# EnricoMiccoli/nodal

Hardware: NVIDIA B200
Metric: unknowns_per_second (higher is better)
Workload: dtype f64

## Files before the change

__graft_entry__.py:

```python
import os
import subprocess
import sys

ROOT = os.path.dirname(os.path.abspath(__file__))
if ROOT not in sys.path:
    sys.path.insert(0, ROOT)


def build():
    subprocess.check_call(["make", "-C", os.path.join(ROOT, "nodal_b200", "csrc"), "-j8"])
    sys.path.insert(0, os.path.join(ROOT, "tests"))
    import helpers
    helpers.stamp_host_lib()
    helpers.amg_host_lib()
    import sources_host
    sources_host.sources_host_lib()
    import amg_cycle_host
    amg_cycle_host.amg_cycle_host_lib()
    ref_nodal = os.path.join(os.environ.get("NODAL_REFERENCE", "/root/reference"), "nodal")
    if os.path.isdir(ref_nodal) and not os.path.isfile(os.path.join(ROOT, "baseline", "_ref", "nodal", "nodal.py")):
        subprocess.call([sys.executable, os.path.join(ROOT, "baseline", "install_ref.py")])
    import nodal_b200
    from nodal_b200 import _lib
    _lib.load()


def smoke():
    import numpy as np
    import nodal_b200 as n
    import nodal_b200.equiv
    from nodal_b200 import dist as ndist
    from nodal_b200 import generators as gen
    from nodal_b200.device import Device
    from oracle import mna_oracle as orc

    N = 24
    r_cpu = orc.equivalent_resistance(orc.grid2d_rows(N), "1", "g", sparse=True, backend="dict")
    r_gpu = n.equiv.equivalent_resistance(gen.grid2d(N), "1", "g", sparse=True)
    r_jac = n.equiv.equivalent_resistance(gen.grid2d(N), "1", "g", sparse=True, precond="jacobi")
    r_amg = n.equiv.equivalent_resistance(gen.grid2d(N), "1", "g", sparse=True, precond="amg", amg={"coarse": 64})
    for r in (r_gpu, r_jac, r_amg):
        assert abs(r - r_cpu) <= 1e-9 * abs(r_cpu), (r, r_cpu)
    dev = Device.get(0)
    import copy
    net = copy.deepcopy(gen.grid2d(64))
    net.process_component(["a1", "A", "1", "1", "g"])
    table = net.table()
    csr, rhs = dev.assemble_csr(table)
    x, info = ndist.single_solver(dev).solve_amg(csr.n, np.array([0, csr.n], dtype=np.int32), csr.indptr, csr.indices,
                                                  csr.data, rhs, rtol=1e-10, gather_below=300)
    r_dist = float(x[net.nodenum["1"]])
    r64 = orc.equivalent_resistance(orc.grid2d_rows(64), "1", "g", sparse=True, backend="dict")
    assert info["status"] == 0 and info["distributed_levels"] >= 1 and abs(r_dist - r64) <= 1e-9 * abs(r64), (info, r_dist, r64)
    pg = gen.power_grid(16, 5, vdd=1.0, load=1e-3, seed=0)
    sol = n.Circuit(pg, sparse=True, eliminate_sources=True).solve()
    red = sol.stats["reduction"]
    assert red["eliminated"] and red["relres_full"] <= 1e-9 and np.all(sol.potentials() <= 1.0), sol.stats
    print(f"smoke ok: R({N}x{N} grid) default={float(r_gpu)!r} jacobi={float(r_jac)!r} amg={float(r_amg)!r} "
          f"oracle={float(r_cpu)!r}; R(64x64) partitioned-AMG form={r_dist!r} oracle={float(r64)!r}; "
          f"power grid 16x16 relres_full={red['relres_full']:.1e}")


if __name__ == "__main__":
    build()
    if len(sys.argv) > 1 and sys.argv[1] == "smoke":
        smoke()
```

include/nodal_b200.h:

```cpp
#ifndef NODAL_B200_H
#define NODAL_B200_H

#include <stdint.h>

#ifdef __cplusplus
extern "C" {
#endif

#define NODAL_ABI_VERSION 1

enum {
    NODAL_OK = 0,
    NODAL_SINGULAR = 1,
    NODAL_NOT_CONVERGED = 2,
    NODAL_BREAKDOWN = 3,
    NODAL_CUDA_ERROR = 4,
    NODAL_BAD_ARG = -1
};

enum { NODAL_T_R = 0, NODAL_T_A = 1, NODAL_T_E = 2, NODAL_T_VCVS = 3, NODAL_T_VCCS = 4,
       NODAL_T_CCVS = 5, NODAL_T_CCCS = 6 };
#define NODAL_GROUND (-1)
#define NODAL_UNUSED (-2)

typedef struct nodal_ctx nodal_ctx;

int nodal_abi_version(void);
const char* nodal_last_error(void);
uint64_t nodal_launch_count(void);
int nodal_ctx_create(int device, nodal_ctx** out);
int nodal_ctx_destroy(nodal_ctx* ctx);
int64_t nodal_ctx_workspace_bytes(nodal_ctx* ctx);

int nodal_stamp_coo(nodal_ctx* ctx, int64_t ncomp,
                    const uint8_t* type, const double* value,
                    const int32_t* a, const int32_t* b, const int32_t* c, const int32_t* d,
                    const int32_t* drv, const int32_t* branch,
                    int32_t kcl, int32_t n, int32_t stride, int32_t colbits,
                    uint64_t* keys, double* vals, void* stream);

int nodal_csr_build(nodal_ctx* ctx, int32_t n, int64_t nslots, int32_t colbits,
                    uint64_t* keys, double* vals, double* rhs,
                    int64_t* nnz_h, void* stream);
int nodal_csr_fetch(nodal_ctx* ctx, int32_t n, int64_t nnz,
                    int32_t* indptr, int32_t* indices, double* data, void* stream);
int nodal_csr_build_ordered(nodal_ctx* ctx, int32_t n, int64_t nslots, int32_t colbits,
                            uint64_t* keys, double* vals, int32_t order, double* rhs, int64_t* nnz_h,
                            void* stream);

int nodal_csr_to_dense(nodal_ctx* ctx, int32_t n, const int32_t* indptr, const int32_t* indices,
                       const double* data, double* G, void* stream);
int nodal_coo_to_dense_atomic(nodal_ctx* ctx, int32_t n, int64_t nslots, int32_t colbits,
                              const uint64_t* keys, const double* vals, double* G, double* rhs,
                              void* stream);

int nodal_spmv(nodal_ctx* ctx, int32_t n, int64_t nnz, const int32_t* indptr,
               const int32_t* indices, const double* data, const double* x, double* y,
               void* stream);

typedef struct nodal_sell nodal_sell;
int nodal_sell_create(nodal_ctx* ctx, int32_t n, int64_t nnz, const int32_t* indptr,
                      const int32_t* indices, const double* data, nodal_sell** out, void* stream);
int nodal_sell_destroy(nodal_sell* m);
int64_t nodal_sell_padded_nnz(const nodal_sell* m);
int nodal_sell_spmv(nodal_ctx* ctx, const nodal_sell* m, const double* x, double* y, void* stream);

int nodal_pcg(nodal_ctx* ctx, int32_t n, int64_t nnz, const int32_t* indptr,
              const int32_t* indices, const double* data, const double* rhs, double* x,
              double rtol, int32_t maxit, int32_t flags,
              int32_t* iters_h, double* relres_h, double* stats_h, void* stream);
#define NODAL_PCG_FORCE_CSR 1
#define NODAL_PCG_NO_GRAPH 2
#define NODAL_PCG_PROFILE 4
#define NODAL_PCG_NO_SCALE 8

int nodal_gmres(nodal_ctx* ctx, int32_t n, int64_t nnz, const int32_t* indptr,
                const int32_t* indices, const double* data, const double* rhs, double* x,
                double rtol, int32_t restart, int32_t maxit,
                int32_t* iters_h, double* relres_h, void* stream);

typedef struct nodal_amg nodal_amg;
int nodal_amg_create(nodal_ctx* ctx, int32_t n, int64_t nnz, const int32_t* indptr,
                     const int32_t* indices, const double* data, const double* params,
                     nodal_amg** out, void* stream);
int nodal_amg_destroy(nodal_amg* amg);
int nodal_amg_info(const nodal_amg* amg, int32_t cap, int32_t* nlevels, int64_t* rows, int64_t* nnz,
                   double* setup_ms, int32_t* direct);
int nodal_amg_fetch_level(nodal_ctx* ctx, const nodal_amg* amg, int32_t level, int32_t* agg,
                          int32_t* indptr, int32_t* indices, double* data, void* stream);
int nodal_amg_apply(nodal_ctx* ctx, const nodal_amg* amg, const double* r, double* z, void* stream);
int nodal_amg_pcg(nodal_ctx* ctx, nodal_amg* amg, const double* rhs, double* x, double rtol,
                  int32_t maxit, int32_t* iters_h, double* relres_h, double* stats_h, void* stream);

int nodal_connected_components(nodal_ctx* ctx, int64_t ncomp, const int32_t* a, const int32_t* b,
                               int32_t kcl, int32_t* labels, int32_t* ncomponents_h,
                               int32_t* reached_h, void* stream);

int nodal_source_forest(nodal_ctx* ctx, int64_t ncomp, const uint8_t* type, const double* value,
                        const int32_t* a, const int32_t* b, const int32_t* branch, int32_t kcl, int32_t be,
                        int32_t* erow, int32_t* adj_ptr, int32_t* adj_row, int32_t* rep_row, double* offset,
                        int32_t* parent_edge, int32_t* depth, int32_t* roots, int64_t* info_h, void* stream);
int nodal_source_reduce_scan(nodal_ctx* ctx, int64_t ncomp, const uint8_t* type, const int32_t* a,
                             const int32_t* b, int32_t kcl, const int32_t* rep_row, const double* offset,
                             uint32_t* pos, int64_t* count_h, void* stream);
int nodal_source_reduce_table(nodal_ctx* ctx, int64_t ncomp, const uint8_t* type, const double* value,
                              const int32_t* a, const int32_t* b, int32_t kcl, const int32_t* rep_row,
                              const double* offset, const uint32_t* pos, uint8_t* out_type, double* out_value,
                              int32_t* out_a, int32_t* out_b, void* stream);
int nodal_source_expand(nodal_ctx* ctx, int32_t kcl, int32_t n, int32_t nsrc, const int32_t* erow,
                        const int32_t* a, const int32_t* b, const int32_t* branch, const int32_t* adj_ptr,
                        const int32_t* adj_row, const int32_t* rep_row, const double* offset,
                        const int32_t* depth, int32_t max_depth, const double* y, const double* rhs,
                        int64_t nnz, const int32_t* indptr, const int32_t* indices, const double* data,
                        double* x, double* relres_h, void* stream);
int nodal_source_potentials(nodal_ctx* ctx, int32_t kcl, int32_t n, const int32_t* rep_row, const double* offset,
                            const double* y, double* x, void* stream);
int nodal_source_tree_rows(nodal_ctx* ctx, int32_t kcl, int32_t n, int64_t nnz_full, int32_t rb, int32_t re,
                           const int32_t* depth, const double* rhs, int64_t nnz, const int32_t* indptr,
                           const int32_t* indices, const double* data, const double* x, int32_t* out_row,
                           double* out_rhs, double* out_gx, int64_t* count_h, void* stream);
int nodal_source_currents(nodal_ctx* ctx, int32_t kcl, int32_t nsrc, const int32_t* erow, const int32_t* a,
                          const int32_t* b, const int32_t* branch, const int32_t* adj_ptr, const int32_t* adj_row,
                          const int32_t* depth, int32_t max_depth, int64_t ntree, const int32_t* tree_row,
                          const double* tree_rhs, const double* tree_gx, double* x, void* stream);
int nodal_source_residual(nodal_ctx* ctx, int32_t n, int64_t nnz_full, int32_t rows, const double* rhs, int64_t nnz,
                          const int32_t* indptr, const int32_t* indices, const double* data, const double* x,
                          double* sums_h, void* stream);

int nodal_lu_solve(nodal_ctx* ctx, int32_t n, double* G, const double* rhs, double* x,
                   int32_t* info_h, void* stream);

int nodal_dgemm_sub_profile(nodal_ctx* ctx, double* C, const double* A, const double* B, int32_t M, int32_t N,
                            int32_t K, int32_t ld, int32_t reps, double* ms_out, void* stream);

int nodal_lu_batched(nodal_ctx* ctx, int64_t batch, int32_t ncomp,
                     const uint8_t* type, const int32_t* a, const int32_t* b,
                     const int32_t* c, const int32_t* d, const int32_t* drv, const int32_t* branch,
                     int32_t kcl, int32_t n, const double* values, double* x, int32_t* info,
                     void* stream);

int nodal_lu_batched_soa(nodal_ctx* ctx, int64_t batch, int32_t ncomp,
                         const uint8_t* type, const int32_t* a, const int32_t* b,
                         const int32_t* c, const int32_t* d, const int32_t* drv, const int32_t* branch,
                         int32_t kcl, int32_t n, const double* values_t, double* x_t, int32_t* info,
                         void* stream);

typedef struct nodal_dist nodal_dist;
int nodal_dist_unique_id(uint8_t id_h[128]);
// ... 54 lines not shown
```

nodal_b200/_lib.py:

```python
from __future__ import annotations

import ctypes as C
import os

_HERE = os.path.dirname(os.path.abspath(__file__))
LIB_PATH = os.path.join(_HERE, "libnodal_b200.so")

OK, SINGULAR, NOT_CONVERGED, BREAKDOWN, CUDA_ERROR, BAD_ARG = 0, 1, 2, 3, 4, -1
PCG_FORCE_CSR, PCG_NO_GRAPH, PCG_PROFILE, PCG_NO_SCALE = 1, 2, 4, 8

_vp, _i32, _i64, _f64 = C.c_void_p, C.c_int32, C.c_int64, C.c_double

SIGNATURES = {
    "nodal_abi_version": (C.c_int, []),
    "nodal_last_error": (C.c_char_p, []),
    "nodal_launch_count": (C.c_uint64, []),
    "nodal_ctx_create": (C.c_int, [C.c_int, C.POINTER(_vp)]),
    "nodal_ctx_destroy": (C.c_int, [_vp]),
    "nodal_ctx_workspace_bytes": (_i64, [_vp]),
    "nodal_stamp_coo": (C.c_int, [_vp, _i64, _vp, _vp, _vp, _vp, _vp, _vp, _vp, _vp,
                                  _i32, _i32, _i32, _i32, _vp, _vp, _vp]),
    "nodal_csr_build": (C.c_int, [_vp, _i32, _i64, _i32, _vp, _vp, _vp, C.POINTER(_i64), _vp]),
    "nodal_csr_build_ordered": (C.c_int, [_vp, _i32, _i64, _i32, _vp, _vp, _i32, _vp, C.POINTER(_i64), _vp]),
    "nodal_csr_fetch": (C.c_int, [_vp, _i32, _i64, _vp, _vp, _vp, _vp]),
    "nodal_csr_to_dense": (C.c_int, [_vp, _i32, _vp, _vp, _vp, _vp, _vp]),
    "nodal_coo_to_dense_atomic": (C.c_int, [_vp, _i32, _i64, _i32, _vp, _vp, _vp, _vp, _vp]),
    "nodal_spmv": (C.c_int, [_vp, _i32, _i64, _vp, _vp, _vp, _vp, _vp, _vp]),
    "nodal_sell_create": (C.c_int, [_vp, _i32, _i64, _vp, _vp, _vp, C.POINTER(_vp), _vp]),
    "nodal_sell_destroy": (C.c_int, [_vp]),
    "nodal_sell_padded_nnz": (_i64, [_vp]),
    "nodal_sell_spmv": (C.c_int, [_vp, _vp, _vp, _vp, _vp]),
    "nodal_pcg": (C.c_int, [_vp, _i32, _i64, _vp, _vp, _vp, _vp, _vp, _f64, _i32, _i32,
                            C.POINTER(_i32), C.POINTER(_f64), C.POINTER(_f64), _vp]),
    "nodal_gmres": (C.c_int, [_vp, _i32, _i64, _vp, _vp, _vp, _vp, _vp, _f64, _i32, _i32,
                              C.POINTER(_i32), C.POINTER(_f64), _vp]),
    "nodal_amg_create": (C.c_int, [_vp, _i32, _i64, _vp, _vp, _vp, C.POINTER(_f64), C.POINTER(_vp), _vp]),
    "nodal_amg_destroy": (C.c_int, [_vp]),
    "nodal_amg_info": (C.c_int, [_vp, _i32, C.POINTER(_i32), C.POINTER(_i64), C.POINTER(_i64),
                                 C.POINTER(_f64), C.POINTER(_i32)]),
    "nodal_amg_fetch_level": (C.c_int, [_vp, _vp, _i32, _vp, _vp, _vp, _vp, _vp]),
    "nodal_amg_apply": (C.c_int, [_vp, _vp, _vp, _vp, _vp]),
    "nodal_amg_pcg": (C.c_int, [_vp, _vp, _vp, _vp, _f64, _i32, C.POINTER(_i32), C.POINTER(_f64),
                                C.POINTER(_f64), _vp]),
    "nodal_connected_components": (C.c_int, [_vp, _i64, _vp, _vp, _i32, _vp, C.POINTER(_i32),
                                             C.POINTER(_i32), _vp]),
    "nodal_source_forest": (C.c_int, [_vp, _i64, _vp, _vp, _vp, _vp, _vp, _i32, _i32] + [_vp] * 8
                            + [C.POINTER(_i64), _vp]),
    "nodal_source_reduce_scan": (C.c_int, [_vp, _i64, _vp, _vp, _vp, _i32, _vp, _vp, _vp, C.POINTER(_i64), _vp]),
    "nodal_source_reduce_table": (C.c_int, [_vp, _i64, _vp, _vp, _vp, _vp, _i32, _vp, _vp, _vp, _vp, _vp, _vp, _vp,
                                            _vp]),
    "nodal_source_expand": (C.c_int, [_vp, _i32, _i32, _i32] + [_vp] * 9 + [_i32, _vp, _vp, _i64, _vp, _vp, _vp, _vp,
                                                                             C.POINTER(_f64), _vp]),
    "nodal_lu_solve": (C.c_int, [_vp, _i32, _vp, _vp, _vp, C.POINTER(_i32), _vp]),
    "nodal_dgemm_sub_profile": (C.c_int, [_vp, _vp, _vp, _vp, _i32, _i32, _i32, _i32, _i32, C.POINTER(_f64), _vp]),
    "nodal_lu_batched": (C.c_int, [_vp, _i64, _i32, _vp, _vp, _vp, _vp, _vp, _vp, _vp,
                                   _i32, _i32, _vp, _vp, _vp, _vp]),
    "nodal_lu_batched_soa": (C.c_int, [_vp, _i64, _i32, _vp, _vp, _vp, _vp, _vp, _vp, _vp,
                                       _i32, _i32, _vp, _vp, _vp, _vp]),
    "nodal_dist_unique_id": (C.c_int, [_vp]),
    "nodal_dist_create": (C.c_int, [_vp, _vp, _i32, _i32, C.POINTER(_vp)]),
    "nodal_dist_create_single": (C.c_int, [_vp, C.POINTER(_vp)]),
    "nodal_dist_destroy": (C.c_int, [_vp]),
    "nodal_dist_pcg": (C.c_int, [_vp, _vp, _i32, _vp, _i64, _vp, _vp, _vp, _vp, _vp, _f64, _i32,
                                 C.POINTER(_i32), C.POINTER(_f64), C.POINTER(_f64), _vp]),
    "nodal_amg_pcg_multi": (C.c_int, [_vp, _vp, _i32, _vp, _vp, _f64, _i32, C.POINTER(_i32), C.POINTER(_f64),
                                      C.POINTER(_i32), _vp]),
    "nodal_amg_profile_sweeps": (C.c_int, [_vp, _vp, _i32, C.POINTER(_f64), _vp]),
    "nodal_amg_profile_cycle": (C.c_int, [_vp, _vp, _i32, C.POINTER(_f64), _vp]),
    "nodal_table_select_scan": (C.c_int, [_vp, _i64, _vp, _vp, _i32, _i32, _vp, C.POINTER(_i64), _vp]),
    "nodal_table_select_gather": (C.c_int, [_vp, _i64, _vp, _i32, _i32] + [_vp] * 16 + [_vp]),
    "nodal_table_select_mna_scan": (C.c_int, [_vp, _i64, _vp, _vp, _vp, _vp, _i32, _i32, _i32, _vp, C.POINTER(_i64),
                                              _vp]),
    "nodal_table_select_mna_gather": (C.c_int, [_vp, _i64, _vp, _i32, _i32, _i32] + [_vp] * 16 + [_vp]),
    "nodal_table_select_type_scan": (C.c_int, [_vp, _i64, _vp, _vp, _vp, _i32, _vp, C.POINTER(_i64), _vp]),
    "nodal_table_select_type_gather": (C.c_int, [_vp, _i64, _vp, _i32] + [_vp] * 16 + [_vp]),
    "nodal_source_potentials": (C.c_int, [_vp, _i32, _i32, _vp, _vp, _vp, _vp, _vp]),
    "nodal_source_tree_rows": (C.c_int, [_vp, _i32, _i32, _i64, _i32, _i32, _vp, _vp, _i64, _vp, _vp, _vp, _vp, _vp,
                                         _vp, _vp, C.POINTER(_i64), _vp]),
    "nodal_source_currents": (C.c_int, [_vp, _i32, _i32] + [_vp] * 7 + [_i32, _i64, _vp, _vp, _vp, _vp, _vp]),
    "nodal_source_residual": (C.c_int, [_vp, _i32, _i64, _i32, _vp, _i64, _vp, _vp, _vp, _vp, C.POINTER(_f64), _vp]),
    "nodal_dist_amg_pcg": (C.c_int, [_vp, _vp, _i32, _vp, _i64, _vp, _vp, _vp, _vp, _vp, C.POINTER(_f64), _f64,
                                     _i32, C.POINTER(_i32), C.POINTER(_f64), C.POINTER(_f64), _vp]),
}

_lib = None


class NodalLibraryError(RuntimeError):
    """The CUDA extension is missing or a CUDA call failed."""


def load():
    global _lib
    if _lib is not None:
        return _lib
    if not os.path.exists(LIB_PATH):
        raise NodalLibraryError(
            f"{LIB_PATH} not found: build it with `python -c 'import __graft_entry__ as g; g.build()'`"
            " (or `make -C nodal_b200/csrc`). nodal_b200 has no CPU fallback.")
    lib = C.CDLL(LIB_PATH)
    for name, (res, args) in SIGNATURES.items():
        fn = getattr(lib, name)
        fn.restype = res
        fn.argtypes = args
    if lib.nodal_abi_version() != 1:
        raise NodalLibraryError("libnodal_b200.so ABI version mismatch")
    _lib = lib
    return lib


def last_error():
    return load().nodal_last_error().decode("utf-8", "replace")


# ... 5 lines not shown
```

nodal_b200/csrc/amg.cu:

```cuda
#include <algorithm>
#include <cmath>

#include "amg_host.cuh"

void amg_free_csr(nodal_ctx* ctx, AmgCsr& a) {
    if (a.owned) {
        ctx_pool_free(ctx, const_cast<int32_t*>(a.indptr));
        ctx_pool_free(ctx, const_cast<int32_t*>(a.indices));
        ctx_pool_free(ctx, const_cast<double*>(a.data));
    }
    a = AmgCsr();
}

int amg_aggregate(nodal_ctx* ctx, int rounds, const AmgCsr& A, int32_t nown, int32_t base,
                  int32_t** agg_out, int32_t* nc_out, cudaStream_t st) {
    const int32_t n = A.n;
    AmgScratch<int32_t> match(ctx, n), best(ctx, n);
    AmgScratch<u32> leader(ctx, n);
    if (!match.ptr || !best.ptr || !leader.ptr) return NODAL_CUDA_ERROR;
    const int grid = amg_rows_grid(ctx, n);
    CUDA_TRY(cudaMemsetAsync(match, 0xFF, sizeof(int32_t) * (size_t)n, st));
    for (int r = 0; r < rounds; ++r) {
        amg_propose_kernel<<<grid, AT, 0, st>>>(n, A.indptr, A.indices, A.data, match, best, nown, base);
        KERNEL_CHECK();
// ... 187 lines not shown
        nodal_set_error("amg: the coarsest operator is not positive definite (pivot %d of %d); "
                        "the matrix is not SPD", *bad_h, n);
        return NODAL_BREAKDOWN;
    }
    return NODAL_OK;
}

int build_hierarchy(nodal_amg* h, int32_t n, int64_t nnz, const int32_t* indptr, const int32_t* indices,
                    const double* data, cudaStream_t st) {
    nodal_ctx* ctx = h->ctx;
    Csr cur;
    cur.n = n; cur.nnz = nnz; cur.indptr = indptr; cur.indices = indices; cur.data = data;
    while (cur.n > h->coarse && (int)h->lv.size() < h->maxlevels) {
        Csr A = cur;
        A.owned = false;
        int32_t* comp = nullptr;
        int rc = NODAL_OK;
        for (int pass = 0; pass < h->passes && rc == NODAL_OK; ++pass) {
            int32_t* agg = nullptr;
            int32_t nc = 0;
            Csr Ac;
            rc = aggregate(h, A, &agg, &nc, st);
            if (rc == NODAL_OK) rc = galerkin(h, A, agg, nc, &Ac, st);
            if (rc == NODAL_OK && comp) {
                amg_compose_kernel<<<rows_grid(ctx, cur.n), AT, 0, st>>>(cur.n, comp, agg);
                ++g_nodal_launches;
                if (cudaGetLastError() != cudaSuccess) {
                    nodal_set_error("amg: amg_compose_kernel launch failed");
                    rc = NODAL_CUDA_ERROR;
                }
            }
            if (!comp) comp = agg;
            else ctx_pool_free(ctx, agg);
            free_csr(ctx, A);
            A = Ac;
        }
        double total_nnz = (double)cur.nnz + (double)A.nnz;
        for (const AmgLevel& P : h->lv) total_nnz += (double)P.nnz;
        const bool too_dense = (double)A.nnz > h->max_fill * (double)cur.nnz ||
                               total_nnz > h->max_complexity * (double)(h->lv.empty() ? cur.nnz : h->lv[0].nnz);
        if (rc != NODAL_OK || (double)A.n > 0.9 * (double)cur.n || too_dense) {
            free_csr(ctx, A);
            ctx_pool_free(ctx, comp);
            if (rc != NODAL_OK) {
                free_csr(ctx, cur);
                return rc;
            }
            break;
        }
        AmgLevel L;
        L.n = cur.n; L.nnz = cur.nnz; L.indptr = cur.indptr; L.indices = cur.indices; L.data = cur.data;
        L.owned = cur.owned;
        L.agg = comp;
        L.nc = A.n;
        h->lv.push_back(L);
        cur = A;
        rc = transpose_pattern(h, h->lv.back(), st);
        if (rc != NODAL_OK) {
            free_csr(ctx, cur);
            return rc;
        }
    }
    AmgLevel L;
    L.n = cur.n; L.nnz = cur.nnz; L.indptr = cur.indptr; L.indices = cur.indices; L.data = cur.data;
    L.owned = cur.owned;
    h->lv.push_back(L);
    for (size_t l = 0; l < h->lv.size(); ++l) {
        AmgLevel& V = h->lv[l];
        NODAL_TRY(sell_from_csr(ctx, V.n, V.nnz, V.indptr, V.indices, V.data, &V.sell, st, nullptr));
        V.x = pool<double>(ctx, V.n);
        V.r = pool<double>(ctx, V.n);
        if (l > 0) V.b = pool<double>(ctx, V.n);
        if (!V.x || !V.r || (l > 0 && !V.b)) return NODAL_CUDA_ERROR;
    }
    if (h->lv.back().n <= h->direct_max) NODAL_TRY(invert_coarsest(h, h->lv.back(), st));
    return NODAL_OK;
}

template <int MODE>
int sell_sweep(const nodal_amg* h, const AmgLevel& V, const double* b, const double* x, double* y,
               double* part, cudaStream_t st) {
    const nodal_sell* m = V.sell;
    amg_sell_kernel<MODE><<<sell_grid(h->ctx, m->nslices), AT, 0, st>>>(
        m->n, m->nslices, m->slice_w, m->cols, m->vals, m->dinv, b, x, h->omega, y, part);
    KERNEL_CHECK();
    return NODAL_OK;
}

template <int MODE>
int cycle_sweep(const nodal_amg* h, const AmgLevel& V, const double* b, const double* xc, double* y,
                cudaStream_t st) {
    const nodal_sell* m = V.sell;
    amg_cycle_sweep_kernel<MODE><<<sell_grid(h->ctx, m->nslices), AT, 0, st>>>(
        m->n, m->nslices, m->slice_w, m->cols, m->vals, m->dinv, b, h->omega, V.agg, xc, h->scale, y);
    KERNEL_CHECK();
    return NODAL_OK;
}

int cycle(const nodal_amg* h, const double* b0, double* z0, cudaStream_t st) {
    const nodal_ctx* ctx = h->ctx;
    const int last = (int)h->lv.size() - 1;
    for (int l = 0; l < last; ++l) {
        const AmgLevel& V = h->lv[l];
        const double* b = l == 0 ? b0 : V.b;
        NODAL_TRY(cycle_sweep<1>(h, V, b, nullptr, V.r, st));
        amg_restrict_kernel<<<rows_grid(ctx, V.nc), AT, 0, st>>>(V.nc, V.pt_ptr, V.pt_idx, V.r,
                                                              h->lv[l + 1].b);
        KERNEL_CHECK();
    }
    {
        const AmgLevel& V = h->lv[last];
        const double* b = last == 0 ? b0 : V.b;
        double* x = last == 0 ? z0 : V.x;
        if (h->inv) amg_gemv_kernel<<<rows_grid(ctx, (int64_t)V.n * 32), AT, 0, st>>>(V.n, h->inv, b, x);
        else amg_jacobi0_kernel<<<rows_grid(ctx, V.n), AT, 0, st>>>(V.n, V.sell->dinv, b, h->omega, x);
        KERNEL_CHECK();
    }
    for (int l = last - 1; l >= 0; --l) {
        const AmgLevel& V = h->lv[l];
        const double* b = l == 0 ? b0 : V.b;
        NODAL_TRY(cycle_sweep<2>(h, V, b, h->lv[l + 1].x, l == 0 ? z0 : V.x, st));
    }
    return NODAL_OK;
}

}

extern "C" int nodal_amg_destroy(nodal_amg* h) {
    if (!h) return NODAL_OK;
    cudaSetDevice(h->device);
    nodal_ctx* ctx = h->ctx;
    for (AmgLevel& V : h->lv) {
        sell_free(V.sell);
        if (V.owned) {
            ctx_pool_free(ctx, const_cast<int32_t*>(V.indptr));
            ctx_pool_free(ctx, const_cast<int32_t*>(V.indices));
            ctx_pool_free(ctx, const_cast<double*>(V.data));
        }
        ctx_pool_free(ctx, V.agg);
        ctx_pool_free(ctx, V.pt_ptr);
        ctx_pool_free(ctx, V.pt_idx);
        ctx_pool_free(ctx, V.b);
        ctx_pool_free(ctx, V.x);
        ctx_pool_free(ctx, V.r);
    }
    ctx_pool_free(ctx, h->inv);
    ctx_pool_free(ctx, h->p);
    ctx_pool_free(ctx, h->q);
    ctx_pool_free(ctx, h->r);
    ctx_pool_free(ctx, h->z);
    ctx_pool_free(ctx, h->part);
    delete h;
    return NODAL_OK;
}

extern "C" int nodal_amg_create(nodal_ctx* ctx, int32_t n, int64_t nnz, const int32_t* indptr,
                                const int32_t* indices, const double* data, const double* params,
                                nodal_amg** out, void* stream) {
    NvtxRange nvtx_range("nodal_amg_create");
    if (!ctx || n < 0 || nnz < 0 || !out) return NODAL_BAD_ARG;
    *out = nullptr;
    cudaStream_t st = (cudaStream_t)stream;
    CUDA_TRY(cudaSetDevice(ctx->device));
    nodal_amg* h = new nodal_amg();
    h->ctx = ctx;
    h->device = ctx->device;
    if (params) {
        if (params[0] >= 1.0) h->passes = (int)params[0];
        if (params[1] >= 1.0) h->coarse = (int)params[1];
        if (params[2] > 0.0) h->omega = params[2];
        if (params[3] > 0.0) h->scale = params[3];
        if (params[4] >= 1.0) h->maxlevels = (int)params[4];
        if (params[5] >= 1.0) h->rounds = (int)params[5];
        if (params[6] >= 1.0) h->direct_max = (int)params[6];
        if (params[7] > 0.0) h->max_fill = params[7];
    }
    cudaEvent_t e0, e1;
// ... 257 lines not shown
```

nodal_b200/csrc/amg_kernels.cuh:

```cuda
#pragma once
#include "amg_core.cuh"
#include "amg_merge_core.cuh"
#include "sparse.cuh"

constexpr int AT = 256;

#define ROW_LOOP(i, n)                                                              \
    for (int64_t i = (int64_t)blockIdx.x * blockDim.x + threadIdx.x; i < (int64_t)(n); \
         i += (int64_t)gridDim.x * blockDim.x)

static __global__ void __launch_bounds__(AT)
amg_propose_kernel(int32_t n, const int32_t* __restrict__ indptr, const int32_t* __restrict__ indices,
                   const double* __restrict__ data, const int32_t* __restrict__ match,
                   int32_t* __restrict__ best, int32_t nown, int32_t base) {
    ROW_LOOP(i, n) best[i] = match[i] >= 0 ? -1 : amg_pick((int32_t)i, indptr, indices, data, match, nown, base);
}

static __global__ void __launch_bounds__(AT)
amg_accept_kernel(int32_t n, const int32_t* __restrict__ best, int32_t* __restrict__ match) {
    ROW_LOOP(i, n) {
        if (match[i] >= 0) continue;
        const int32_t b = best[i];
        if (b >= 0 && best[b] == (int32_t)i) match[i] = b;
    }
// ... 19 lines not shown
static __global__ void __launch_bounds__(AT)
amg_compose_kernel(int32_t n, int32_t* __restrict__ comp, const int32_t* __restrict__ next) {
    ROW_LOOP(i, n) comp[i] = next[comp[i]];
}

static __global__ void __launch_bounds__(AT)
amg_relabel_kernel(int32_t n, const int32_t* __restrict__ indptr, const int32_t* __restrict__ indices,
                   const double* __restrict__ data, const int32_t* __restrict__ agg, int cb,
                   u64* __restrict__ keys, double* __restrict__ vals) {
    ROW_LOOP(i, n) {
        const u64 hi = (u64)agg[i] << cb;
        const int32_t e = indptr[i + 1];
        for (int32_t p = indptr[i]; p < e; ++p) {
            keys[p] = hi | (u64)agg[indices[p]];
            vals[p] = data[p];
        }
    }
}

static __global__ void __launch_bounds__(AT)
amg_pt_keys_kernel(int32_t n, const int32_t* __restrict__ agg, int cb, u64* __restrict__ keys,
                   double* __restrict__ vals) {
    ROW_LOOP(i, n) {
        keys[i] = ((u64)agg[i] << cb) | (u64)i;
        vals[i] = 1.0;
    }
}

static __global__ void __launch_bounds__(AT)
amg_dense_init_kernel(int32_t n, const int32_t* __restrict__ indptr, const int32_t* __restrict__ indices,
                      const double* __restrict__ data, double* __restrict__ M) {
    const int64_t W = 2 * (int64_t)n;
    ROW_LOOP(i, n) {
        M[i * W + n + i] = 1.0;
        const int32_t e = indptr[i + 1];
        for (int32_t p = indptr[i]; p < e; ++p) M[i * W + indices[p]] = data[p];
    }
}

static __global__ void __launch_bounds__(AT)
amg_gj_step_kernel(int32_t n, int32_t k, const double* __restrict__ src, double* __restrict__ dst,
                   int* __restrict__ bad) {
    const int64_t W = 2 * (int64_t)n;
    const double piv = src[k * W + k];
    if (blockIdx.x == 0 && threadIdx.x == 0 && !(piv > 0.0) && *bad == 0) *bad = k + 1;
    ROW_LOOP(idx, (int64_t)n * W) {
        const int64_t i = idx / W, j = idx - i * W;
        const double rkj = src[k * W + j] / piv;
        dst[idx] = i == k ? rkj : src[idx] - src[i * W + k] * rkj;
    }
}

static __global__ void __launch_bounds__(AT)
amg_dense_extract_kernel(int32_t n, const double* __restrict__ M, double* __restrict__ inv) {
    const int64_t W = 2 * (int64_t)n;
    ROW_LOOP(idx, (int64_t)n * n) {
        const int64_t i = idx / n, j = idx - i * n;
        inv[idx] = M[i * W + n + j];
    }
}

static __global__ void __launch_bounds__(AT)
amg_gemv_kernel(int32_t n, const double* __restrict__ inv, const double* __restrict__ b,
                double* __restrict__ x) {
    const int lane = threadIdx.x & 31;
    const int64_t warp = ((int64_t)blockIdx.x * blockDim.x + threadIdx.x) >> 5;
    const int64_t nwarps = ((int64_t)gridDim.x * blockDim.x) >> 5;
    for (int64_t r = warp; r < n; r += nwarps) {
        double acc = 0.0;
        for (int32_t j = lane; j < n; j += 32) acc = fma(inv[r * n + j], b[j], acc);
        acc = warp_sum(acc);
        if (lane == 0) x[r] = acc;
    }
}

static __global__ void __launch_bounds__(AT)
amg_jacobi0_kernel(int32_t n, const double* __restrict__ dinv, const double* __restrict__ b,
                   double omega, double* __restrict__ x) {
    ROW_LOOP(i, n) x[i] = amg_jacobi_start(omega, dinv[i], b[i]);
}

template <int MODE>
static __global__ void __launch_bounds__(AT, 5)
amg_sell_kernel(int32_t n, int32_t nslices, const u32* __restrict__ slice_w,
                const int32_t* __restrict__ cols, const double* __restrict__ vals,
                const double* __restrict__ dinv, const double* __restrict__ b,
                const double* __restrict__ x, double omega, double* __restrict__ y,
                double* __restrict__ part) {
    __shared__ double red[33];
    const int lane = threadIdx.x & 31;
    const int64_t warp = ((int64_t)blockIdx.x * blockDim.x + threadIdx.x) >> 5;
    const int64_t nwarps = ((int64_t)gridDim.x * blockDim.x) >> 5;
    double dot = 0.0;
    for (int64_t s = warp; s < nslices; s += nwarps) {
        const u32 w0 = slice_w[s];
        const int w = (int)(slice_w[s + 1] - w0);
        const double acc = sell_row_dot(cols, vals, (int64_t)w0 * 32 + lane, w, x);
        const int64_t r = s * 32 + lane;
        if (r < n) {
            if (MODE == 0) { y[r] = acc; dot = fma(x[r], acc, dot); }
            if (MODE == 1) y[r] = amg_residual(b[r], acc);
            if (MODE == 2) y[r] = amg_jacobi_update(omega, dinv[r], b[r], acc, x[r]);
        }
    }
    if (MODE == 0) {
        const double t = block_sum(dot, red);
        if (threadIdx.x == 0) part[blockIdx.x] = t;
    }
}

static __global__ void __launch_bounds__(AT)
amg_restrict_kernel(int32_t nc, const int32_t* __restrict__ pt_ptr, const int32_t* __restrict__ pt_idx,
                    const double* __restrict__ r, double* __restrict__ bc) {
    ROW_LOOP(I, nc) {
        double s = 0.0;
        const int32_t e = pt_ptr[I + 1];
        for (int32_t p = pt_ptr[I]; p < e; ++p) s += r[pt_idx[p]];
        bc[I] = s;
    }
}

static __global__ void __launch_bounds__(AT)
amg_prolong_kernel(int32_t n, const int32_t* __restrict__ agg, const double* __restrict__ xc,
                   double scale, const double* __restrict__ x, double* __restrict__ xa) {
    ROW_LOOP(i, n) xa[i] = amg_prolong_add(scale, xc[agg[i]], x[i]);
}

struct JacobiStartAt {
    const double* __restrict__ dinv;
    const double* __restrict__ b;
    double omega;
    __device__ __forceinline__ double operator()(int32_t c) const {
        return amg_jacobi_start(omega, __ldg(&dinv[c]), __ldg(&b[c]));
    }
};

struct ProlongatedAt {
    JacobiStartAt x0;
    const int32_t* __restrict__ agg;
    const double* __restrict__ xc;
    double scale;
    __device__ __forceinline__ double operator()(int32_t c) const {
        return amg_prolong_add(scale, __ldg(&xc[__ldg(&agg[c])]), x0(c));
    }
};

template <int MODE>
static __global__ void __launch_bounds__(AT, 5)
amg_cycle_sweep_kernel(int32_t n, int32_t nslices, const u32* __restrict__ slice_w,
                       const int32_t* __restrict__ cols, const double* __restrict__ vals,
                       const double* __restrict__ dinv, const double* __restrict__ b, double omega,
                       const int32_t* __restrict__ agg, const double* __restrict__ xc, double scale,
                       double* __restrict__ y) {
    const int lane = threadIdx.x & 31;
    const int64_t warp = ((int64_t)blockIdx.x * blockDim.x + threadIdx.x) >> 5;
    const int64_t nwarps = ((int64_t)gridDim.x * blockDim.x) >> 5;
    const JacobiStartAt x0{dinv, b, omega};
    const ProlongatedAt xa{x0, agg, xc, scale};
    for (int64_t s = warp; s < nslices; s += nwarps) {
        const u32 w0 = slice_w[s];
        const int w = (int)(slice_w[s + 1] - w0);
        const int64_t base = (int64_t)w0 * 32 + lane;
        const int64_t r = s * 32 + lane;
        if (MODE == 1) {
            const double acc = sell_row_gather(cols, vals, base, w, x0);
            if (r < n) y[r] = amg_residual(b[r], acc);
        }
        if (MODE == 2) {
            const double acc = sell_row_gather(cols, vals, base, w, xa);
            if (r < n) y[r] = amg_jacobi_update(omega, dinv[r], b[r], acc, xa((int32_t)r));
        }
    }
}

static __global__ void __launch_bounds__(AT)
apcg_dot_kernel(int32_t n, const double* __restrict__ a, const double* __restrict__ b,
                double* __restrict__ part) {
    __shared__ double red[33];
    double t = 0.0;
    ROW_LOOP(i, n) t = fma(a[i], b[i], t);
    t = block_sum(t, red);
    if (threadIdx.x == 0) part[blockIdx.x] = t;
}

static __global__ void __launch_bounds__(AT)
apcg_sum_kernel(const double* __restrict__ part, int count, double* __restrict__ out) {
    __shared__ double red[33];
    const double t = reduce_partials(part, count, red);
    if (threadIdx.x == 0) out[0] = t;
}

static __global__ void __launch_bounds__(AT)
apcg_update_kernel(int32_t n, const double* __restrict__ part_pq, int npq, const double* __restrict__ rz,
                   const double* __restrict__ p, const double* __restrict__ q, double* __restrict__ x,
                   double* __restrict__ r, double* __restrict__ part_rr) {
    __shared__ double red[33];
    const double pq = reduce_partials(part_pq, npq, red);
    const double alpha = rz[0] / pq;
    double t = 0.0;
    ROW_LOOP(i, n) {
        x[i] = fma(alpha, p[i], x[i]);
        const double ri = fma(-alpha, q[i], r[i]);
        r[i] = ri;
        t = fma(ri, ri, t);
    }
    t = block_sum(t, red);
    if (threadIdx.x == 0) part_rr[blockIdx.x] = t;
}

static __global__ void __launch_bounds__(AT)
apcg_direction_kernel(int32_t n, const double* __restrict__ part_rz, int nrz,
                      const double* __restrict__ rz_old, double* __restrict__ rz_new,
                      const double* __restrict__ z, double* __restrict__ p, int first) {
    __shared__ double red[33];
    const double rzn = reduce_partials(part_rz, nrz, red);
    const double beta = first ? 0.0 : rzn / rz_old[0];
    ROW_LOOP(i, n) p[i] = first ? z[i] : fma(beta, p[i], z[i]);
    if (blockIdx.x == 0 && threadIdx.x == 0) rz_new[0] = rzn;
}


static __global__ void __launch_bounds__(AT)
amg_count_members_kernel(int32_t n, const int32_t* __restrict__ agg, u32* __restrict__ cnt) {
    ROW_LOOP(i, n) atomicAdd(&cnt[agg[i]], 1u);
}

static __global__ void __launch_bounds__(AT)
amg_place_members_kernel(int32_t n, const int32_t* __restrict__ agg, const int32_t* __restrict__ pt_ptr,
                         u32* __restrict__ cursor, int32_t* __restrict__ pt_idx) {
    ROW_LOOP(i, n) {
        const int32_t a = agg[i];
        pt_idx[pt_ptr[a] + (int32_t)atomicAdd(&cursor[a], 1u)] = (int32_t)i;
    }
}

static __global__ void __launch_bounds__(AT)
amg_sort_members_kernel(int32_t nc, const int32_t* __restrict__ pt_ptr, int32_t* __restrict__ pt_idx) {
    ROW_LOOP(I, nc) {
        const int32_t b = pt_ptr[I], e = pt_ptr[I + 1];
        for (int32_t p = b + 1; p < e; ++p) {
            const int32_t v = pt_idx[p];
            int32_t q = p;
            while (q > b && pt_idx[q - 1] > v) { pt_idx[q] = pt_idx[q - 1]; --q; }
            pt_idx[q] = v;
        }
    }
}

static __global__ void __launch_bounds__(AT)
amg_merge_bound_kernel(int32_t nc, const int32_t* __restrict__ pt_ptr, const int32_t* __restrict__ pt_idx,
                       const int32_t* __restrict__ indptr, u32* __restrict__ bound) {
    ROW_LOOP(I, nc) bound[I] = (u32)amg_merge_bound((int32_t)I, pt_ptr, pt_idx, indptr);
// ... 37 lines not shown
```

nodal_b200/csrc/amg_multi.cu:

```cuda
#include <algorithm>
#include <cmath>

#include "amg_host.cuh"

namespace {

constexpr int MK = 8;

template <int W>
__device__ __forceinline__ void sell_dot_fixed_multi(const int32_t* __restrict__ cols, const double* __restrict__ vals,
                                                     int64_t base, const double* __restrict__ x, int64_t stride, int K,
                                                     double* acc) {
    int32_t c[W];
    double v[W];
#pragma unroll
    for (int i = 0; i < W; ++i) {
        c[i] = cols[base + (int64_t)i * 32];
        v[i] = vals[base + (int64_t)i * 32];
    }
#pragma unroll
    for (int k = 0; k < 8; ++k) {
        if (k < K) {
            const double* xk = x + (int64_t)k * stride;
            double a = acc[k];
#pragma unroll
            for (int i = 0; i < W; ++i) a = fma(v[i], __ldg(&xk[c[i]]), a);
            acc[k] = a;
        }
    }
}

__device__ __forceinline__ void sell_row_dot_multi(const int32_t* __restrict__ cols, const double* __restrict__ vals,
                                                   int64_t base, int w, const double* __restrict__ x, int64_t stride,
                                                   int K, double* acc) {
    int k = 0;
    for (; k + 4 <= w; k += 4) sell_dot_fixed_multi<4>(cols, vals, base + (int64_t)k * 32, x, stride, K, acc);
    const int64_t b = base + (int64_t)k * 32;
    switch (w - k) {
        case 3: sell_dot_fixed_multi<3>(cols, vals, b, x, stride, K, acc); break;
        case 2: sell_dot_fixed_multi<2>(cols, vals, b, x, stride, K, acc); break;
        case 1: sell_dot_fixed_multi<1>(cols, vals, b, x, stride, K, acc); break;
        default: break;
    }
}

template <int MODE>
__global__ void __launch_bounds__(AT, 3)
amgm_sell_kernel(int32_t n, int32_t nslices, const u32* __restrict__ slice_w, const int32_t* __restrict__ cols,
                 const double* __restrict__ vals, const double* __restrict__ dinv, const double* __restrict__ b,
                 const double* __restrict__ x, double omega, double* __restrict__ y, double* __restrict__ part, int K,
                 int nparts) {
    __shared__ double red[33];
    const int lane = threadIdx.x & 31;
    const int64_t warp = ((int64_t)blockIdx.x * blockDim.x + threadIdx.x) >> 5;
    const int64_t nwarps = ((int64_t)gridDim.x * blockDim.x) >> 5;
    double dot[MK];
#pragma unroll
    for (int k = 0; k < MK; ++k) dot[k] = 0.0;
    for (int64_t s = warp; s < nslices; s += nwarps) {
        const u32 w0 = slice_w[s];
        const int w = (int)(slice_w[s + 1] - w0);
        double acc[MK];
#pragma unroll
        for (int k = 0; k < MK; ++k) acc[k] = 0.0;
        sell_row_dot_multi(cols, vals, (int64_t)w0 * 32 + lane, w, x, n, K, acc);
        const int64_t r = s * 32 + lane;
        if (r < n) {
            const double di = MODE == 2 ? dinv[r] : 0.0;
#pragma unroll
            for (int k = 0; k < MK; ++k) {
                if (k >= K) break;
                const int64_t o = (int64_t)k * n + r;
                if (MODE == 0) { y[o] = acc[k]; dot[k] = fma(x[o], acc[k], dot[k]); }
                if (MODE == 1) y[o] = b[o] - acc[k];
                if (MODE == 2) y[o] = x[o] + omega * di * (b[o] - acc[k]);
            }
        }
    }
    if (MODE == 0) {
#pragma unroll
        for (int k = 0; k < MK; ++k) {
            if (k < K) {
                const double t = block_sum(dot[k], red);
                if (threadIdx.x == 0) part[(size_t)k * nparts + blockIdx.x] = t;
            }
        }
    }
}

__global__ void __launch_bounds__(AT)
amgm_jacobi0_kernel(int32_t n, int K, const double* __restrict__ dinv, const double* __restrict__ b, double omega,
                    double* __restrict__ x) {
    ROW_LOOP(i, n) {
        const double d = omega * dinv[i];
        for (int k = 0; k < K; ++k) x[(int64_t)k * n + i] = d * b[(int64_t)k * n + i];
    }
}

__global__ void __launch_bounds__(AT)
amgm_restrict_kernel(int32_t n, int32_t nc, int K, const int32_t* __restrict__ pt_ptr, const int32_t* __restrict__ pt_idx,
                     const double* __restrict__ r, double* __restrict__ bc) {
    ROW_LOOP(I, nc) {
        const int32_t b0 = pt_ptr[I], e = pt_ptr[I + 1];
        for (int k = 0; k < K; ++k) {
            double s = 0.0;
            for (int32_t p = b0; p < e; ++p) s += r[(int64_t)k * n + pt_idx[p]];
            bc[(int64_t)k * nc + I] = s;
        }
    }
}

__global__ void __launch_bounds__(AT)
amgm_prolong_kernel(int32_t n, int32_t nc, int K, const int32_t* __restrict__ agg, const double* __restrict__ xc,
                    double scale, const double* __restrict__ x, double* __restrict__ xa) {
    ROW_LOOP(i, n) {
        const int32_t a = agg[i];
        for (int k = 0; k < K; ++k) xa[(int64_t)k * n + i] = x[(int64_t)k * n + i] + scale * xc[(int64_t)k * nc + a];
    }
}

__global__ void __launch_bounds__(AT)
amgm_gemv_kernel(int32_t n, int K, const double* __restrict__ inv, const double* __restrict__ b, double* __restrict__ x) {
    const int lane = threadIdx.x & 31;
    const int64_t warp = ((int64_t)blockIdx.x * blockDim.x + threadIdx.x) >> 5;
    const int64_t nwarps = ((int64_t)gridDim.x * blockDim.x) >> 5;
    for (int64_t t = warp; t < (int64_t)n * K; t += nwarps) {
        const int64_t k = t / n, r = t - k * n;
        double acc = 0.0;
        for (int32_t j = lane; j < n; j += 32) acc = fma(inv[r * n + j], b[k * n + j], acc);
        acc = warp_sum(acc);
        if (lane == 0) x[k * n + r] = acc;
    }
}

__global__ void __launch_bounds__(AT)
amgm_dot_kernel(int32_t n, int K, const double* __restrict__ a, const double* __restrict__ b, double* __restrict__ part,
                int nparts) {
    __shared__ double red[33];
    for (int k = 0; k < K; ++k) {
        double t = 0.0;
        ROW_LOOP(i, n) t = fma(a[(int64_t)k * n + i], b[(int64_t)k * n + i], t);
        t = block_sum(t, red);
        if (threadIdx.x == 0) part[(size_t)k * nparts + blockIdx.x] = t;
    }
}

__global__ void __launch_bounds__(AT)
amgm_sum_kernel(const double* __restrict__ part, int count, int nparts, int K, double* __restrict__ out) {
    __shared__ double red[33];
    for (int k = 0; k < K; ++k) {
        const double t = reduce_partials(part + (size_t)k * nparts, count, red);
        if (threadIdx.x == 0) out[k] = t;
    }
}

__global__ void __launch_bounds__(AT)
amgm_update_kernel(int32_t n, int K, const double* __restrict__ part_pq, int npq, int nparts, const double* __restrict__ rz,
                   const int* __restrict__ active, const double* __restrict__ p, const double* __restrict__ q,
                   double* __restrict__ x, double* __restrict__ r, double* __restrict__ part_rr) {
    __shared__ double red[33];
    for (int k = 0; k < K; ++k) {
        const double pq = reduce_partials(part_pq + (size_t)k * nparts, npq, red);
        const bool on = active[k] != 0;
        const double alpha = on ? rz[k] / pq : 0.0;
        double t = 0.0;
        ROW_LOOP(i, n) {
            const int64_t o = (int64_t)k * n + i;
            double ri = r[o];
            if (on) {
                x[o] = fma(alpha, p[o], x[o]);
                ri = fma(-alpha, q[o], ri);
                r[o] = ri;
            }
            t = fma(ri, ri, t);
        }
        t = block_sum(t, red);
        if (threadIdx.x == 0) part_rr[(size_t)k * nparts + blockIdx.x] = t;
    }
}

__global__ void __launch_bounds__(AT)
amgm_direction_kernel(int32_t n, int K, const double* __restrict__ part_rz, int nrz, int nparts,
                      const double* __restrict__ rz_old, double* __restrict__ rz_new, const int* __restrict__ active,
                      const double* __restrict__ z, double* __restrict__ p, int first) {
    __shared__ double red[33];
    for (int k = 0; k < K; ++k) {
        const double rzn = reduce_partials(part_rz + (size_t)k * nparts, nrz, red);
        const bool on = active[k] != 0;
        const double beta = first ? 0.0 : rzn / rz_old[k];
        if (on) {
            ROW_LOOP(i, n) {
                const int64_t o = (int64_t)k * n + i;
                p[o] = first ? z[o] : fma(beta, p[o], z[o]);
            }
        }
        if (blockIdx.x == 0 && threadIdx.x == 0) rz_new[k] = on ? rzn : rz_old[k];
    }
}

struct Work {
    std::vector<double*> x, r, b;
    double *p = nullptr, *q = nullptr, *rr = nullptr, *z = nullptr, *part = nullptr, *scal = nullptr;
    int* active = nullptr;
    std::vector<void*> owned;
};

template <int MODE>
int sweep(const nodal_amg* h, const AmgLevel& V, int K, const double* b, const double* x, double* y, double* part,
          int nparts, cudaStream_t st) {
    const nodal_sell* m = V.sell;
    amgm_sell_kernel<MODE><<<amg_sell_grid(h->ctx, m->nslices), AT, 0, st>>>(
        m->n, m->nslices, m->slice_w, m->cols, m->vals, m->dinv, b, x, h->omega, y, part, K, nparts);
    KERNEL_CHECK();
    return NODAL_OK;
}

int cycle_multi(const nodal_amg* h, Work& W, int K, const double* b0, double* z0, cudaStream_t st) {
    const nodal_ctx* ctx = h->ctx;
    const int last = (int)h->lv.size() - 1;
    for (int l = 0; l < last; ++l) {
        const AmgLevel& V = h->lv[l];
        const double* b = l == 0 ? b0 : W.b[l];
        amgm_jacobi0_kernel<<<amg_rows_grid(ctx, V.n), AT, 0, st>>>(V.n, K, V.sell->dinv, b, h->omega, W.x[l]);
        KERNEL_CHECK();
        NODAL_TRY(sweep<1>(h, V, K, b, W.x[l], W.r[l], nullptr, 0, st));
        amgm_restrict_kernel<<<amg_rows_grid(ctx, V.nc), AT, 0, st>>>(V.n, V.nc, K, V.pt_ptr, V.pt_idx, W.r[l], W.b[l + 1]);
        KERNEL_CHECK();
    }
    {
        const AmgLevel& V = h->lv[last];
        const double* b = last == 0 ? b0 : W.b[last];
        double* x = last == 0 ? z0 : W.x[last];
        if (h->inv) amgm_gemv_kernel<<<amg_rows_grid(ctx, (int64_t)V.n * 32 * K), AT, 0, st>>>(V.n, K, h->inv, b, x);
        else amgm_jacobi0_kernel<<<amg_rows_grid(ctx, V.n), AT, 0, st>>>(V.n, K, V.sell->dinv, b, h->omega, x);
        KERNEL_CHECK();
    }
    for (int l = last - 1; l >= 0; --l) {
        const AmgLevel& V = h->lv[l];
        const double* b = l == 0 ? b0 : W.b[l];
        double* xa = W.r[l];
        amgm_prolong_kernel<<<amg_rows_grid(ctx, V.n), AT, 0, st>>>(V.n, V.nc, K, V.agg, W.x[l + 1], h->scale, W.x[l], xa);
        KERNEL_CHECK();
        NODAL_TRY(sweep<2>(h, V, K, b, xa, l == 0 ? z0 : W.x[l], nullptr, 0, st));
    }
    return NODAL_OK;
}

}

extern "C" int nodal_amg_pcg_multi(nodal_ctx* ctx, nodal_amg* h, int32_t K, const double* rhs, double* x, double rtol,
                                   int32_t maxit, int32_t* iters_h, double* relres_h, int32_t* status_h, void* stream) {
    if (!ctx || !h || h->ctx != ctx || K < 1 || K > MK || !iters_h || !relres_h || !status_h) return NODAL_BAD_ARG;
    NvtxRange nvtx_range("nodal_amg_pcg_multi");
    for (int k = 0; k < K; ++k) { iters_h[k] = 0; relres_h[k] = 0.0; status_h[k] = NODAL_OK; }
    if (h->lv.empty()) return NODAL_OK;
    cudaStream_t st = (cudaStream_t)stream;
    CUDA_TRY(cudaSetDevice(ctx->device));
    const AmgLevel& A = h->lv[0];
    const int32_t n = A.n;
    const int gv = amg_rows_grid(ctx, n), gs = amg_sell_grid(ctx, A.sell->nslices);
    const int nparts = std::max(gv, gs);
    Work W;
    auto alloc = [&](size_t count) -> double* {
        double* p = amg_pool<double>(ctx, count);
        if (p) W.owned.push_back(p);
        return p;
    };
    auto run = [&]() -> int {
        const int L = (int)h->lv.size();
        W.x.assign(L, nullptr); W.r.assign(L, nullptr); W.b.assign(L, nullptr);
        for (int l = 0; l < L; ++l) {
            const size_t len = (size_t)K * h->lv[l].n + 2;
            W.x[l] = alloc(len);
            W.r[l] = alloc(len);
            if (l > 0) W.b[l] = alloc(len);
            if (!W.x[l] || !W.r[l] || (l > 0 && !W.b[l])) return NODAL_CUDA_ERROR;
        }
        const size_t vlen = (size_t)K * n + 2;
        W.p = alloc(vlen); W.q = alloc(vlen); W.rr = alloc(vlen); W.z = alloc(vlen);
        W.part = alloc(3 * (size_t)MK * nparts + 8);
        W.scal = alloc(4 * MK + 8);
        W.active = reinterpret_cast<int*>(alloc(MK));
        if (!W.p || !W.q || !W.rr || !W.z || !W.part || !W.scal || !W.active) return NODAL_CUDA_ERROR;
        double* part_pq = W.part;
        double* part_rr = W.part + (size_t)MK * nparts;
        double* part_rz = W.part + 2 * (size_t)MK * nparts;
        double* rz[2] = {W.scal, W.scal + MK};
        double* norms = W.scal + 2 * MK;
        double* host = reinterpret_cast<double*>(static_cast<char*>(ctx->pinned) + 2048);
        int* host_active = reinterpret_cast<int*>(host + MK);

        auto norms_to_host = [&](const double* a, const double* b, double* out) -> int {
            amgm_dot_kernel<<<gv, AT, 0, st>>>(n, K, a, b, part_rr, nparts);
            KERNEL_CHECK();
            amgm_sum_kernel<<<1, AT, 0, st>>>(part_rr, gv, nparts, K, norms);
            KERNEL_CHECK();
            CUDA_TRY(cudaMemcpyAsync(host, norms, sizeof(double) * K, cudaMemcpyDeviceToHost, st));
            CUDA_TRY(cudaStreamSynchronize(st));
            for (int k = 0; k < K; ++k) out[k] = host[k];
            return NODAL_OK;
        };
        double bb[MK], rrv[MK], bnorm[MK];
        int active[MK], iters[MK];
        NODAL_TRY(norms_to_host(rhs, rhs, bb));
        NODAL_TRY(sweep<1>(h, A, K, rhs, x, W.rr, nullptr, 0, st));
        NODAL_TRY(norms_to_host(W.rr, W.rr, rrv));
        int remaining = 0;
        for (int k = 0; k < K; ++k) {
            iters[k] = 0;
            bnorm[k] = sqrt(bb[k]);
            if (!(bb[k] > 0.0)) {
                active[k] = 0;
                status_h[k] = bb[k] == 0.0 ? NODAL_OK : NODAL_BREAKDOWN;
                relres_h[k] = 0.0;
                if (bb[k] == 0.0) CUDA_TRY(cudaMemsetAsync(x + (size_t)k * n, 0, sizeof(double) * (size_t)n, st));
                continue;
            }
            relres_h[k] = sqrt(rrv[k]) / bnorm[k];
            active[k] = relres_h[k] > rtol ? 1 : 0;
            remaining += active[k];
        }
        auto push_active = [&]() -> int {
            for (int k = 0; k < MK; ++k) host_active[k] = k < K ? active[k] : 0;
            CUDA_TRY(cudaMemcpyAsync(W.active, host_active, sizeof(int) * MK, cudaMemcpyHostToDevice, st));
            return NODAL_OK;
        };
        if (remaining) {
            NODAL_TRY(push_active());
            int par = 0;
            NODAL_TRY(cycle_multi(h, W, K, W.rr, W.z, st));
// ... 50 lines not shown
```

nodal_b200/csrc/dist.cu:

```cuda
#include <algorithm>
#include <chrono>
#include <vector>

#include "dist_common.cuh"
#include "pcg_kernels.cuh"

NcclApi g_nccl;

int load_nccl() {
    if (g_nccl.handle) return NODAL_OK;
    void* h = dlopen("libnccl.so.2", RTLD_NOW | RTLD_GLOBAL);
    if (!h) h = dlopen("libnccl.so", RTLD_NOW | RTLD_GLOBAL);
    if (!h) {
        nodal_set_error("cannot dlopen libnccl.so.2: %s", dlerror());
        return NODAL_CUDA_ERROR;
    }
#define SYM(field, name)                                                      \
    g_nccl.field = reinterpret_cast<decltype(g_nccl.field)>(dlsym(h, name)); \
    if (!g_nccl.field) {                                                      \
        nodal_set_error("libnccl: missing symbol %s", name);                  \
        return NODAL_CUDA_ERROR;                                              \
    }
    SYM(GetUniqueId, "ncclGetUniqueId")
    SYM(CommInitRank, "ncclCommInitRank")
// ... 501 lines not shown
                if (need_cnt[threadIdx.x] > 0) {
                    const long long t0 = clock64();
                    while (ld_sys_u64(&mine->hflag[threadIdx.x]) < tag) {
                        if (clock64() - t0 > P2P_SPIN_LIMIT) {
                            dev->done = 1; dev->status = NODAL_CUDA_ERROR; mine->err = 1;
                            break;
                        }
                    }
                }
            }
            __threadfence_system();
            __syncthreads();
            if (threadIdx.x == 0) {
                const unsigned long long tv2 = gtime();
                sy->dbg[0] += tv1 - tv0; sy->dbg[1] += tv2 - tv1; sy->dbg[2] += 1;
            }
        }
    }
    {
        const int64_t n2 = n >> 1;
        const int64_t stride = (int64_t)gridDim.x * blockDim.x;
        double2* x2 = reinterpret_cast<double2*>(x);
        double2* r2 = reinterpret_cast<double2*>(r);
        double2* p2 = reinterpret_cast<double2*>(p);
        double2* s2 = reinterpret_cast<double2*>(s);
        double2* u2 = reinterpret_cast<double2*>(u);
        const double2* w2 = reinterpret_cast<const double2*>(w);
        const double2* d2 = reinterpret_cast<const double2*>(dinv);
        const uchar2* m2 = reinterpret_cast<const uchar2*>(bmask);
        for (int64_t i = (int64_t)blockIdx.x * blockDim.x + threadIdx.x; i < n2; i += stride) {
            const uchar2 mk = m2[i];
            double2 xv = x2[i], rv = r2[i], pv = p2[i], sv = s2[i];
            const double2 wv = w2[i];
            double2 dv = make_double2(1.0, 1.0);
            if (!UNIT) dv = d2[i];
            if (mk.x | mk.y) {
                if (!mk.x) {
                    pv.x = fma(beta, pv.x, dv.x * rv.x); sv.x = fma(beta, sv.x, wv.x);
                    xv.x = fma(alpha, pv.x, xv.x); rv.x = fma(-alpha, sv.x, rv.x);
                    p[2 * i] = pv.x; s[2 * i] = sv.x; x[2 * i] = xv.x; r[2 * i] = rv.x;
                    if (!UNIT) { const double uv = dv.x * rv.x; u[2 * i] = uv; lg = fma(rv.x, uv, lg); }
                    lrr = fma(rv.x, rv.x, lrr);
                }
                if (!mk.y) {
                    pv.y = fma(beta, pv.y, dv.y * rv.y); sv.y = fma(beta, sv.y, wv.y);
                    xv.y = fma(alpha, pv.y, xv.y); rv.y = fma(-alpha, sv.y, rv.y);
                    p[2 * i + 1] = pv.y; s[2 * i + 1] = sv.y; x[2 * i + 1] = xv.y; r[2 * i + 1] = rv.y;
                    if (!UNIT) { const double uv = dv.y * rv.y; u[2 * i + 1] = uv; lg = fma(rv.y, uv, lg); }
                    lrr = fma(rv.y, rv.y, lrr);
                }
                continue;
            }
            pv.x = fma(beta, pv.x, dv.x * rv.x); pv.y = fma(beta, pv.y, dv.y * rv.y);
            sv.x = fma(beta, sv.x, wv.x);        sv.y = fma(beta, sv.y, wv.y);
            xv.x = fma(alpha, pv.x, xv.x);       xv.y = fma(alpha, pv.y, xv.y);
            rv.x = fma(-alpha, sv.x, rv.x);      rv.y = fma(-alpha, sv.y, rv.y);
            p2[i] = pv; s2[i] = sv; x2[i] = xv; r2[i] = rv;
            if (!UNIT) {
                double2 uv;
                uv.x = dv.x * rv.x; uv.y = dv.y * rv.y;
                u2[i] = uv;
                lg = fma(rv.x, uv.x, lg); lg = fma(rv.y, uv.y, lg);
            }
            lrr = fma(rv.x, rv.x, lrr); lrr = fma(rv.y, rv.y, lrr);
        }
        if ((n & 1) && blockIdx.x == 0 && threadIdx.x == 0 && !bmask[n - 1]) {
            const int64_t i = n - 1;
            const double dvi = UNIT ? 1.0 : dinv[i];
            const double pv = fma(beta, p[i], dvi * r[i]);
            const double sv = fma(beta, s[i], w[i]);
            const double rv = fma(-alpha, sv, r[i]);
            p[i] = pv; s[i] = sv; x[i] = fma(alpha, pv, x[i]); r[i] = rv;
            if (!UNIT) { const double uv = dvi * rv; u[i] = uv; lg = fma(rv, uv, lg); }
            lrr = fma(rv, rv, lrr);
        }
    }
    lrr = block_sum(lrr, sm);
    lg = UNIT ? lrr : block_sum(lg, sm);
    if (threadIdx.x == 0) { part_g[blockIdx.x] = lg; part_rr[blockIdx.x] = lrr; }
}

__global__ void __launch_bounds__(PCG_THREADS, 5)
dist_spmv_allreduce_sell_kernel(PcgDev* __restrict__ dev, int32_t n, int32_t nslices,
                                const u32* __restrict__ slice_w, const int32_t* __restrict__ cols,
                                const double* __restrict__ vals, const double* __restrict__ u,
                                double* __restrict__ w, double* part_d, const double* __restrict__ part_g,
                                const double* __restrict__ part_rr, int cnt_v, DistSync* sy,
                                unsigned long long* seq, int R, int me,
                                char* const* __restrict__ peer, double* __restrict__ out) {
    __shared__ double sm[40];
    __shared__ double s_slot[P2P_MAXR][3];
    __shared__ int s_flag;
    if (block_done(&dev->done)) return;
    const unsigned long long s0 = *seq;
    const unsigned long long tag = s0 + 1;
    P2PMail* mine = reinterpret_cast<P2PMail*>(peer[me]);
    if (blockIdx.x == 0 && threadIdx.x == 0) {
        const unsigned long long now = gtime();
        sy->dbg[12] += now - sy->dbg[8];
        sy->dbg[9] = now;
    }
    const int lane = threadIdx.x & 31;
    const int64_t warp = ((int64_t)blockIdx.x * blockDim.x + threadIdx.x) >> 5;
    const int64_t nwarps = ((int64_t)gridDim.x * blockDim.x) >> 5;
    double dot = 0.0;
    for (int64_t s = warp; s < nslices; s += nwarps) {
        const u32 w0 = slice_w[s];
        const int wd = (int)(slice_w[s + 1] - w0);
        const int64_t base = (int64_t)w0 * 32 + lane;
        const double acc = sell_row_dot(cols, vals, base, wd, u);
        const int64_t row = s * 32 + lane;
        if (row < n) {
            w[row] = acc;
            dot = fma(acc, __ldg(&u[row]), dot);
        }
    }
    dot = block_sum(dot, sm);
    if (threadIdx.x == 0) part_d[blockIdx.x] = dot;
    if (!last_cta_arrive(sy->ticket_s, &s_flag)) return;
    const unsigned long long ts0 = gtime();
    double g, rr, dl;
    reduce3_cg(part_g, cnt_v, part_rr, cnt_v, part_d, (int)gridDim.x, sm, g, rr, dl);
    const int par = (int)(s0 & 1ull);
    __syncthreads();
    if (threadIdx.x == 0) s_flag = 0;
    __syncthreads();
    const unsigned long long ts1 = gtime();
    unsigned long long ts2 = ts1;
    if (threadIdx.x < R) {
        P2PMail* m = reinterpret_cast<P2PMail*>(peer[threadIdx.x]);
        volatile double* slot = m->red[par][me];
        slot[0] = g; slot[1] = dl; slot[2] = rr;
        st_sys_u64(reinterpret_cast<unsigned long long*>(&m->red[par][me][3]), tag);
        ts2 = gtime();
        const unsigned long long* tp = reinterpret_cast<const unsigned long long*>(&mine->red[par][threadIdx.x][3]);
        const long long t0 = clock64();
        while (ld_sys_u64(tp) != tag) {
            if (clock64() - t0 > P2P_SPIN_LIMIT) { s_flag = 1; break; }
        }
        const volatile double* in = mine->red[par][threadIdx.x];
        s_slot[threadIdx.x][0] = in[0]; s_slot[threadIdx.x][1] = in[1]; s_slot[threadIdx.x][2] = in[2];
    }
    __syncthreads();
    if (threadIdx.x == 0) {
        if (s_flag) {
            dev->done = 1; dev->status = NODAL_CUDA_ERROR; mine->err = 1;
        } else {
            double sg = 0.0, sd = 0.0, sr = 0.0;
            for (int t = 0; t < R; ++t) { sg += s_slot[t][0]; sd += s_slot[t][1]; sr += s_slot[t][2]; }
            out[0] = sg; out[1] = sd; out[2] = sr;
            *seq = tag;
            if (dev->iters >= dev->maxit) { dev->done = 1; dev->status = NODAL_NOT_CONVERGED; }
        }
        const unsigned long long ts3 = gtime();
        sy->dbg[4] += ts1 - ts0; sy->dbg[5] += ts2 - ts1; sy->dbg[6] += ts3 - ts2; sy->dbg[7] += 1;
        sy->dbg[13] += ts0 - sy->dbg[9];
        sy->dbg[10] = ts3;
    }
}

__global__ void __launch_bounds__(DT)
dist_mark_rows_kernel(int64_t m, const int32_t* __restrict__ rows, unsigned char* __restrict__ mask) {
    for (int64_t i = (int64_t)blockIdx.x * blockDim.x + threadIdx.x; i < m; i += (int64_t)gridDim.x * blockDim.x)
        mask[rows[i]] = 1;
}

static int grid_of(nodal_ctx* ctx, int64_t work) {
    int64_t b = (work + DT - 1) / DT;
    const int64_t cap = (int64_t)ctx->num_sms * 8;
    return (int)std::max<int64_t>(1, std::min(b, cap));
}

int peer_heap_ensure(nodal_ctx* ctx, nodal_dist* d, PeerHeap* hp, size_t bytes, size_t zero_bytes,
                     cudaStream_t st, bool* usable) {
    *usable = false;
    const int R = d->nranks, me = d->rank;
    if (R < 2 || R > P2P_MAXR || d->p2p_disabled || getenv("NODAL_DIST_NO_P2P")) return NODAL_OK;
    int* flag_dev = nullptr;
    CUDA_TRY(cudaMalloc(&flag_dev, 256));
    int ok = 1;
    if (hp->bytes < bytes) {
        CUDA_TRY(cudaStreamSynchronize(st));
        peer_heap_release(d, hp);
        const size_t want = align_up(bytes + bytes / 4, 2 << 20);
        cudaIpcMemHandle_t mine;
        char* handles_dev = nullptr;
        std::vector<cudaIpcMemHandle_t> all((size_t)R);
        if (cudaMalloc(&hp->shm, want) != cudaSuccess) ok = 0;
        if (ok && cudaMemset(hp->shm, 0, std::min(zero_bytes, want)) != cudaSuccess) ok = 0;
        if (ok && cudaIpcGetMemHandle(&mine, hp->shm) != cudaSuccess) ok = 0;
        if (!ok) memset(&mine, 0, sizeof(mine));
        (void)cudaGetLastError();
        CUDA_TRY(cudaMalloc(&handles_dev, sizeof(cudaIpcMemHandle_t) * (size_t)(R + 1)));
// ... 318 lines not shown
            const int64_t want = ((int64_t)nloc * A.tpr + PCG_THREADS - 1) / PCG_THREADS;
            A.g1 = (int)std::min<int64_t>((int64_t)ctx->num_sms * 8, want);
        }
        const bool fused = p2p && A.sell && getenv("NODAL_DIST_NO_FUSE") == nullptr;
        const int gmax = std::max(A.g1, g2) + 1;
        const size_t vloc = align_up(sizeof(double) * (size_t)nloc, 256);
        const size_t vext = align_up(sizeof(double) * (size_t)(nloc + nhalo + 2), 256);
        NODAL_TRY(ctx_reserve(ctx, 7 * vloc + 2 * vext + 8 * align_up(sizeof(double) * gmax, 256) + 8192));
        double* ext = p2p ? reinterpret_cast<double*>(d->pcg.shm + P2P_HDR)
                          : carve<double>(ctx, (size_t)nloc + nhalo + 2);
        double* r = unit ? ext : carve<double>(ctx, nloc);
        double* u = ext;
        double* q = carve<double>(ctx, nloc);
        double* p = carve<double>(ctx, nloc);
        double* s = carve<double>(ctx, nloc);
        double* w = carve<double>(ctx, nloc);
        double* bh = unit ? carve<double>(ctx, nloc) : nullptr;
        if (unit && !bh) return NODAL_CUDA_ERROR;
        double* xe = carve<double>(ctx, (size_t)nloc + nhalo + 2);
        double* part_g = carve<double>(ctx, gmax);
        double* part_d = carve<double>(ctx, gmax);
        double* part_rr = carve<double>(ctx, gmax);
        double* part_bb = carve<double>(ctx, gmax);
        double* SC = carve<double>(ctx, 16);
        PcgDev* dev = carve<PcgDev>(ctx, 1);
        double* dinv_own = A.sell ? nullptr : carve<double>(ctx, nloc);
        if (!r || !q || !p || !s || !w || !u || !xe || !part_bb || !SC || !dev) return NODAL_CUDA_ERROR;
        const double* dinv = A.sell ? sell->dinv : dinv_own;
        if (dinv_own) {
            csr_dinv_kernel<<<g2, PCG_THREADS, 0, st>>>(nloc, indptr, lcols, data, dinv_own);
            KERNEL_CHECK();
        }
        CUDA_TRY(cudaMemsetAsync(dev, 0, sizeof(PcgDev), st));
        CUDA_TRY(cudaMemsetAsync(SC, 0, sizeof(double) * 16, st));
        const double* b_eff = rhs_local;
        if (unit) {
            pcg_scale_vec_kernel<<<g2, PCG_THREADS, 0, st>>>(nloc, rhs_local, sc, bh, 0);
            KERNEL_CHECK();
            pcg_scale_vec_kernel<<<g2, PCG_THREADS, 0, st>>>(nloc, x_local, sc, x_local, 1);
            KERNEL_CHECK();
            b_eff = bh;
        }

        auto spmv_plain = [&](const double* in, double* out) -> int {
            if (A.sell) return nodal_sell_spmv(ctx, A.sell, in, out, st);
            return csr_spmv_launch(ctx, nloc, nnz, indptr, lcols, data, in, out, st);
        };
        auto start = [&](int first) -> int {
            cgcg_reset_kernel<<<1, 32, 0, st>>>(dev);
            KERNEL_CHECK();
            CUDA_TRY(cudaMemcpyAsync(xe, x_local, sizeof(double) * (size_t)nloc, cudaMemcpyDeviceToDevice, st));
            NODAL_TRY(exchange(xe, st));
            NODAL_TRY(spmv_plain(xe, q));
            if (unit)
                cgcg_start_kernel<true><<<g2, PCG_THREADS, 0, st>>>(nloc, b_eff, q, dinv, r, u, p, s, part_g, part_rr, part_bb);
            else
                cgcg_start_kernel<false><<<g2, PCG_THREADS, 0, st>>>(nloc, b_eff, q, dinv, r, u, p, s, part_g, part_rr, part_bb);
            KERNEL_CHECK();
            NODAL_TRY(exchange(ext, st));
            NODAL_TRY(launch_k1(A, dev, ext, w, part_d, st));
            cgcg_reduce_kernel<<<1, PCG_THREADS, 0, st>>>(dev, part_g, part_rr, part_bb, g2, part_d, A.g1, SC, 1);
            KERNEL_CHECK();
            if (R > 1) NCCL_TRY(g_nccl.AllReduce(SC, SC, 4, ncclFloat64, ncclSum, d->comm, st));
            cgcg_scalars_kernel<<<1, 32, 0, st>>>(dev, SC, rtol, maxit, first);
            KERNEL_CHECK();
            return NODAL_OK;
        };
        auto iteration = [&](int par, cudaStream_t sx) -> int {
            double* cur = SC + par * 4;
            double* nxt = SC + (par ^ 1) * 4;
            if (fused) {
                if (unit)
                    dist_vector_push_kernel<true><<<g2, PCG_THREADS, 0, sx>>>(
                        dev, nloc, cur, nxt, x_local, r, p, s, w, dinv, u, part_g, part_rr, sy, d->pcg.seq, R, me,
                        send_idx, send_off_dev, dest_off_dev, need_cnt_dev, blist_dev, nb_rows, nbc, push_rng_dev,
                        bmask_dev, d->pcg.peer_dev);
                else
                    dist_vector_push_kernel<false><<<g2, PCG_THREADS, 0, sx>>>(
                        dev, nloc, cur, nxt, x_local, r, p, s, w, dinv, u, part_g, part_rr, sy, d->pcg.seq, R, me,
                        send_idx, send_off_dev, dest_off_dev, need_cnt_dev, blist_dev, nb_rows, nbc, push_rng_dev,
                        bmask_dev, d->pcg.peer_dev);
                KERNEL_CHECK();
                dist_spmv_allreduce_sell_kernel<<<A.g1, PCG_THREADS, 0, sx>>>(
                    dev, nloc, sell->nslices, sell->slice_w, sell->cols, sell->vals, ext, w, part_d, part_g,
                    part_rr, g2, sy, d->pcg.seq, R, me, d->pcg.peer_dev, nxt);
                KERNEL_CHECK();
                return NODAL_OK;
            }
            if (unit)
                cgcg_vector_kernel<true><<<g2, PCG_THREADS, 0, sx>>>(dev, nloc, cur, nxt, x_local, r, p, s, w, dinv, u,
                                                                    part_g, part_rr);
            else
                cgcg_vector_kernel<false><<<g2, PCG_THREADS, 0, sx>>>(dev, nloc, cur, nxt, x_local, r, p, s, w, dinv, u,
                                                                     part_g, part_rr);
            KERNEL_CHECK();
            if (p2p) {
                p2p_push_kernel<<<1, 1024, 0, sx>>>(dev, d->pcg.seq, R, me, send_idx, send_off_dev, dest_off_dev,
                                                    d->pcg.peer_dev, ext);
                KERNEL_CHECK();
                p2p_wait_halo_kernel<<<1, 32, 0, sx>>>(dev, d->pcg.seq, R, me, need_cnt_dev,
                                                       reinterpret_cast<P2PMail*>(d->pcg.shm));
                KERNEL_CHECK();
            } else {
                NODAL_TRY(exchange(ext, sx));
            }
            NODAL_TRY(launch_k1(A, dev, ext, w, part_d, sx));
            if (p2p) {
                p2p_reduce_kernel<<<1, PCG_THREADS, 0, sx>>>(dev, d->pcg.seq, R, me, part_g, part_rr, g2, part_d, A.g1,
                                                            d->pcg.peer_dev, nxt);
                KERNEL_CHECK();
            } else {
                cgcg_reduce_kernel<<<1, PCG_THREADS, 0, sx>>>(dev, part_g, part_rr, nullptr, g2, part_d, A.g1, nxt, 0);
                KERNEL_CHECK();
                if (R > 1) NCCL_TRY(g_nccl.AllReduce(nxt, nxt, 3, ncclFloat64, ncclSum, d->comm, sx));
            }
            return NODAL_OK;
        };

        NODAL_TRY(start(1));
        const int CH = 32;
        const bool use_graph = getenv("NODAL_DIST_NO_GRAPH") == nullptr;
        if (use_graph) {
            const auto c0 = std::chrono::steady_clock::now();
            const unsigned long long before = g_nodal_launches;
            CUDA_TRY(cudaStreamCreateWithFlags(&cap, cudaStreamNonBlocking));
            if (A.sell) NODAL_TRY(sell_set_l2_window(ctx, A.sell, cap));
            CUDA_TRY(cudaStreamBeginCapture(cap, cudaStreamCaptureModeThreadLocal));
            int crc = NODAL_OK;
            for (int i = 0; i < CH && crc == NODAL_OK; ++i) crc = iteration(i & 1, cap);
            cudaError_t ce = cudaStreamEndCapture(cap, &graph);
            if (crc != NODAL_OK) return crc;
            CUDA_TRY(ce);
            CUDA_TRY(cudaGraphInstantiate(&gexec, graph, 0));
            launches_per_chunk = g_nodal_launches - before;
            g_nodal_launches = before;
            host_ms_capture = std::chrono::duration<double, std::milli>(std::chrono::steady_clock::now() - c0).count();
        }
        CUDA_TRY(cudaEventRecord(ev1, st));
        PcgDev* poll = reinterpret_cast<PcgDev*>(ctx->pinned);
        double last_true_rr = -1.0;
        for (;;) {
            const int64_t max_chunks = (int64_t)maxit / CH + 3;
            int64_t k = 0;
            for (;; ++k) {
                if (use_graph) {
                    CUDA_TRY(cudaGraphLaunch(gexec, st));
                    g_nodal_launches += launches_per_chunk;
                } else {
                    for (int i = 0; i < CH; ++i) NODAL_TRY(iteration(i & 1, st));
                }
                CUDA_TRY(cudaMemcpyAsync(&poll[k & 1], dev, sizeof(PcgDev), cudaMemcpyDeviceToHost, st));
                CUDA_TRY(cudaEventRecord(ev_poll[k & 1], st));
                if (k >= 1) {
                    CUDA_TRY(cudaEventSynchronize(ev_poll[(k - 1) & 1]));
                    if (poll[(k - 1) & 1].done) break;
                }
                if (k > max_chunks) break;
            }
            CUDA_TRY(cudaStreamSynchronize(st));
            host = poll[k & 1];
            if (!host.done) host.status = NODAL_NOT_CONVERGED;
            if (host.status == NODAL_BREAKDOWN) break;
            const int recurrence_status = host.status;
            const int iters_so_far = host.iters;
            NODAL_TRY(start(0));
            CUDA_TRY(cudaMemcpyAsync(&poll[0], dev, sizeof(PcgDev), cudaMemcpyDeviceToHost, st));
            CUDA_TRY(cudaStreamSynchronize(st));
// ... 101 lines not shown
```

nodal_b200/csrc/dist_amg.cu:

```cuda
#include <algorithm>
#include <chrono>
#include <cmath>
#include <memory>
#include <vector>

#include "amg_host.cuh"
#include "dist_common.cuh"
#include "pcg_kernels.cuh"

namespace {

constexpr int DA = 256;
constexpr size_t AMG_HDR = 8192;
constexpr int AMG_SLOTS = 60;
struct AmgMail {
    double red[2][P2P_MAXR][4];
    unsigned long long rtag[2][P2P_MAXR];
    unsigned long long flag[AMG_SLOTS][P2P_MAXR];
    unsigned long long cnt[AMG_SLOTS];
    unsigned int ticket[AMG_SLOTS];
    unsigned long long rseq;
    unsigned long long err;
};
static_assert(sizeof(AmgMail) <= AMG_HDR, "mailbox must fit the header");
// ... 111 lines not shown
        for (int o = 0; o < R; ++o) {
            double* dst = reinterpret_cast<double*>(peer[o] + voff) + dest_off[o];
            for (int64_t j = gtid; j < nown; j += gstride) dst[j] = src[j];
        }
    }
    __syncthreads();
    if (threadIdx.x == 0) {
        __threadfence_system();
        const unsigned int t = atomicAdd(&mine->ticket[slot], 1u);
        s_last = (t == gridDim.x - 1);
        if (s_last) mine->ticket[slot] = 0;
    }
    __syncthreads();
    if (!s_last) return;
    __threadfence_system();
    if (threadIdx.x < R && threadIdx.x != me) {
        const bool sends = mode == 1 ? nown > 0 : send_off[threadIdx.x + 1] > send_off[threadIdx.x];
        if (sends) st_sys_u64(&reinterpret_cast<AmgMail*>(peer[threadIdx.x])->flag[slot][me], tag);
        if (need_cnt[threadIdx.x] > 0) {
            const long long t0 = clock64();
            while (ld_sys_u64(&mine->flag[slot][threadIdx.x]) < tag) {
                if (clock64() - t0 > P2P_SPIN_LIMIT) { mine->err = 1; break; }
            }
        }
    }
    __threadfence_system();
    __syncthreads();
    if (threadIdx.x == 0) mine->cnt[slot] = tag;
}

__global__ void __launch_bounds__(DA)
acg_vector_kernel(PcgDev* __restrict__ dev, int32_t n, double* __restrict__ cur, const double* __restrict__ prev,
                  double* __restrict__ x, double* __restrict__ r, double* __restrict__ p, double* __restrict__ s,
                  const double* __restrict__ u, const double* __restrict__ w, double* __restrict__ part_rr) {
    __shared__ double sm[40];
    if (block_done(&dev->done)) return;
    const double g = cur[0], dl = cur[1], rr = cur[2];
    const double gp = prev[0], ap = prev[3];
    const bool conv = rr <= dev->tol2;
    double beta = 0.0, den = dl;
    if (ap != 0.0) { beta = g / gp; den = dl - beta * g / ap; }
    const double alpha = g / den;
    const bool bad = !(den > 0.0) || !(rr == rr) || !(g == g);
    if (blockIdx.x == 0 && threadIdx.x == 0) {
        dev->rr = rr;
        if (conv) { dev->done = 1; dev->status = NODAL_OK; }
        else if (bad) { dev->done = 1; dev->status = NODAL_BREAKDOWN; }
        else { dev->iters = dev->iters + 1; cur[3] = alpha; }
    }
    if (conv || bad) return;
    double lrr = 0.0;
    const int64_t n2 = n >> 1;
    double2* x2 = reinterpret_cast<double2*>(x);
    double2* r2 = reinterpret_cast<double2*>(r);
    double2* p2 = reinterpret_cast<double2*>(p);
    double2* s2 = reinterpret_cast<double2*>(s);
    const double2* u2 = reinterpret_cast<const double2*>(u);
    const double2* w2 = reinterpret_cast<const double2*>(w);
    GRID_LOOP(i, n2) {
        double2 pv = p2[i], sv = s2[i], rv = r2[i], xv = x2[i];
        const double2 uv = u2[i], wv = w2[i];
        pv.x = fma(beta, pv.x, uv.x);   pv.y = fma(beta, pv.y, uv.y);
        sv.x = fma(beta, sv.x, wv.x);   sv.y = fma(beta, sv.y, wv.y);
        rv.x = fma(-alpha, sv.x, rv.x); rv.y = fma(-alpha, sv.y, rv.y);
        xv.x = fma(alpha, pv.x, xv.x);  xv.y = fma(alpha, pv.y, xv.y);
        p2[i] = pv; s2[i] = sv; r2[i] = rv; x2[i] = xv;
        lrr = fma(rv.x, rv.x, lrr);
        lrr = fma(rv.y, rv.y, lrr);
    }
    if ((n & 1) && blockIdx.x == 0 && threadIdx.x == 0) {
        const int64_t i = n - 1;
        const double pv = fma(beta, p[i], u[i]);
        const double sv = fma(beta, s[i], w[i]);
        const double rv = fma(-alpha, sv, r[i]);
        p[i] = pv; s[i] = sv; r[i] = rv;
        x[i] = fma(alpha, pv, x[i]);
        lrr = fma(rv, rv, lrr);
    }
    lrr = block_sum(lrr, sm);
    if (threadIdx.x == 0) part_rr[blockIdx.x] = lrr;
}

__global__ void __launch_bounds__(DA, 5)
acg_spmv_dots_kernel(int32_t n, int32_t nslices, const u32* __restrict__ slice_w, const int32_t* __restrict__ cols,
                     const double* __restrict__ vals, const double* __restrict__ u, const double* __restrict__ r,
                     double* __restrict__ w, double* __restrict__ part_g, double* __restrict__ part_d) {
    __shared__ double sm[40];
    const int lane = threadIdx.x & 31;
    const int64_t warp = ((int64_t)blockIdx.x * blockDim.x + threadIdx.x) >> 5;
    const int64_t nwarps = ((int64_t)gridDim.x * blockDim.x) >> 5;
    double lg = 0.0, ld = 0.0;
    for (int64_t s = warp; s < nslices; s += nwarps) {
        const u32 w0 = slice_w[s];
        const int wd = (int)(slice_w[s + 1] - w0);
        const double acc = sell_row_dot(cols, vals, (int64_t)w0 * 32 + lane, wd, u);
        const int64_t row = s * 32 + lane;
        if (row < n) {
            const double uv = __ldg(&u[row]);
            w[row] = acc;
            lg = fma(r[row], uv, lg);
            ld = fma(acc, uv, ld);
        }
    }
    lg = block_sum(lg, sm);
    ld = block_sum(ld, sm);
    if (threadIdx.x == 0) { part_g[blockIdx.x] = lg; part_d[blockIdx.x] = ld; }
}

__global__ void __launch_bounds__(DA)
acg_start_kernel(int32_t n, const double* __restrict__ b, const double* __restrict__ r,
                 double* __restrict__ p, double* __restrict__ s, double* __restrict__ part_rr, double* __restrict__ part_bb) {
    __shared__ double sm[40];
    double lrr = 0.0, lbb = 0.0;
    GRID_LOOP(i, n) {
        const double bv = b[i], rv = r[i];
        p[i] = 0.0; s[i] = 0.0;
        lrr = fma(rv, rv, lrr);
        lbb = fma(bv, bv, lbb);
    }
    lrr = block_sum(lrr, sm);
    lbb = block_sum(lbb, sm);
    if (threadIdx.x == 0) { part_rr[blockIdx.x] = lrr; part_bb[blockIdx.x] = lbb; }
}

__global__ void __launch_bounds__(DA)
acg_allreduce_kernel(PcgDev* __restrict__ dev, int check_done, const double* __restrict__ a, int na,
                     const double* __restrict__ b, int nb, const double* __restrict__ c, int nc,
                     const double* __restrict__ d4, int nd, int R, int me, char* const* __restrict__ peer,
                     int use_mail, double* __restrict__ out, int enforce_maxit) {
    __shared__ double sm[40];
    __shared__ int s_timeout;
    if (check_done && block_done(&dev->done)) return;
    const double va = a ? reduce_partials(a, na, sm) : 0.0;
    const double vb = b ? reduce_partials(b, nb, sm) : 0.0;
    const double vc = c ? reduce_partials(c, nc, sm) : 0.0;
    const double vd = d4 ? reduce_partials(d4, nd, sm) : 0.0;
    if (!use_mail) {
        if (threadIdx.x == 0) {
            out[0] = va; out[1] = vb; out[2] = vc; out[3] = vd;
            if (enforce_maxit && dev->iters >= dev->maxit) { dev->done = 1; dev->status = NODAL_NOT_CONVERGED; }
        }
        return;
    }
    AmgMail* mine = reinterpret_cast<AmgMail*>(peer[me]);
    const unsigned long long s0 = *reinterpret_cast<volatile unsigned long long*>(&mine->rseq);
    const unsigned long long tag = s0 + 1;
    const int par = (int)(s0 & 1ull);
    if (threadIdx.x == 0) s_timeout = 0;
    __syncthreads();
    if (threadIdx.x < R) {
        AmgMail* m = reinterpret_cast<AmgMail*>(peer[threadIdx.x]);
        volatile double* slot = m->red[par][me];
        slot[0] = va; slot[1] = vb; slot[2] = vc; slot[3] = vd;
        __threadfence_system();
        st_sys_u64(&m->rtag[par][me], tag);
        const long long t0 = clock64();
        while (ld_sys_u64(&mine->rtag[par][threadIdx.x]) != tag) {
            if (clock64() - t0 > P2P_SPIN_LIMIT) { s_timeout = 1; break; }
        }
    }
    __threadfence_system();
    __syncthreads();
    if (threadIdx.x == 0) {
        if (s_timeout) {
            dev->done = 1; dev->status = NODAL_CUDA_ERROR; mine->err = 1;
        } else {
            double t0 = 0.0, t1 = 0.0, t2 = 0.0, t3 = 0.0;
            for (int t = 0; t < R; ++t) {
                const volatile double* slot = mine->red[par][t];
                t0 += slot[0]; t1 += slot[1]; t2 += slot[2]; t3 += slot[3];
            }
            out[0] = t0; out[1] = t1; out[2] = t2; out[3] = t3;
            mine->rseq = tag;
            if (enforce_maxit && dev->iters >= dev->maxit) { dev->done = 1; dev->status = NODAL_NOT_CONVERGED; }
        }
    }
}

// ... 368 lines not shown
        S.owned.push_back(L.pt_idx);
        have_members = true;
        NODAL_TRY(amg_galerkin_merge(ctx, loc, L.pt_ptr, L.pt_idx, ncur, lab32, 0x7fffffff, next, st));
    } else {
        AmgScratch<u64> keys(ctx, (size_t)std::max<int64_t>(nnz, 1));
        AmgScratch<double> vals(ctx, (size_t)std::max<int64_t>(nnz, 1));
        if (!keys.ptr || !vals.ptr) return NODAL_CUDA_ERROR;
        const int cb = amg_bit_length(nc_glob);
        da_relabel_global_kernel<<<amg_rows_grid(ctx, nloc), DA, 0, st>>>(nloc, L.A.indptr, L.lcols, L.A.data, lab, cb, keys, vals);
        KERNEL_CHECK();
        NODAL_TRY(build_rows(S, nc_glob, nnz, cb, keys, vals, (*next_bounds)[S.me], ncur, next));
    }
    {
        std::vector<int32_t> fine_k, coarse_k;
        NODAL_TRY(gather_counts(S, (int32_t)(nnz >> 10) + 1, fine_k));
        NODAL_TRY(gather_counts(S, (int32_t)(next->nnz >> 10) + 1, coarse_k));
        S.nnz_k_total += (double)coarse_k[S.R];
        if (S.nnz_k_fine == 0.0) { S.nnz_k_fine = (double)fine_k[S.R]; S.nnz_k_total += S.nnz_k_fine; }
        if ((double)coarse_k[S.R] > S.max_fill * (double)fine_k[S.R] || S.nnz_k_total > S.max_complexity * S.nnz_k_fine) {
            amg_free_csr(ctx, *next);
            ctx_pool_free(ctx, comp);
            *stalled = true;
            return NODAL_OK;
        }
    }
    L.agg = comp;
    S.owned.push_back(comp);
    L.nc = ncur;
    if (!have_members) {
        NODAL_TRY(amg_transpose_pattern(ctx, nloc, comp, &L.pt_ptr, &L.pt_idx, st));
        S.owned.push_back(L.pt_ptr);
        S.owned.push_back(L.pt_idx);
    }
    return NODAL_OK;
}

int gather_operator(Solver& S, const AmgCsr& A, const std::vector<int32_t>& bounds, AmgCsr* out) {
    nodal_ctx* ctx = S.ctx;
    cudaStream_t st = S.st;
    const int R = S.R, me = S.me;
    if (R == 1) { *out = A; out->owned = false; return NODAL_OK; }
    if (A.nnz >= ((int64_t)1 << 31)) return NODAL_BAD_ARG;
    std::vector<int32_t> nzb;
    NODAL_TRY(gather_counts(S, (int32_t)A.nnz, nzb));
    const int32_t n = bounds[R];
    const int64_t nnz = nzb[R];
    AmgScratch<int32_t> ip(ctx, (size_t)n + 1), ix(ctx, (size_t)std::max<int64_t>(nnz, 1));
    AmgScratch<double> dv(ctx, (size_t)std::max<int64_t>(nnz, 1));
    if (!ip.ptr || !ix.ptr || !dv.ptr) return NODAL_CUDA_ERROR;
    const int32_t nloc = bounds[me + 1] - bounds[me];
    CUDA_TRY(cudaMemcpyAsync(ip.ptr + bounds[me], A.indptr, sizeof(int32_t) * (size_t)nloc, cudaMemcpyDeviceToDevice, st));
    if (A.nnz) {
        CUDA_TRY(cudaMemcpyAsync(ix.ptr + nzb[me], A.indices, sizeof(int32_t) * (size_t)A.nnz, cudaMemcpyDeviceToDevice, st));
        CUDA_TRY(cudaMemcpyAsync(dv.ptr + nzb[me], A.data, sizeof(double) * (size_t)A.nnz, cudaMemcpyDeviceToDevice, st));
    }
    NCCL_TRY(g_nccl.GroupStart());
    for (int o = 0; o < R; ++o) {
        const int32_t rows = bounds[o + 1] - bounds[o], cnt = nzb[o + 1] - nzb[o];
        if (rows) NCCL_TRY(g_nccl.Broadcast(ip.ptr + bounds[o], ip.ptr + bounds[o], rows, ncclInt32, o, S.d->comm, st));
        if (cnt) {
            NCCL_TRY(g_nccl.Broadcast(ix.ptr + nzb[o], ix.ptr + nzb[o], cnt, ncclInt32, o, S.d->comm, st));
            NCCL_TRY(g_nccl.Broadcast(dv.ptr + nzb[o], dv.ptr + nzb[o], cnt, ncclFloat64, o, S.d->comm, st));
        }
    }
    NCCL_TRY(g_nccl.GroupEnd());
    for (int o = 0; o < R; ++o) {
        const int32_t rows = bounds[o + 1] - bounds[o];
        if (rows && nzb[o]) {
            da_offset_indptr_kernel<<<amg_rows_grid(ctx, rows), DA, 0, st>>>(rows, ip.ptr + bounds[o], nzb[o]);
            KERNEL_CHECK();
        }
    }
    da_set_i32_kernel<<<1, 32, 0, st>>>(ip.ptr + n, (int32_t)nnz);
    KERNEL_CHECK();
    out->n = n; out->nnz = nnz; out->owned = true;
    out->indptr = ip.keep(); out->indices = ix.keep(); out->data = dv.keep();
    return NODAL_OK;
}

template <int MODE>
int sweep(Solver& S, const DLevel& L, const double* b, const double* x, double* y, cudaStream_t sx) {
    const nodal_sell* m = L.sell;
    amg_sell_kernel<MODE><<<amg_sell_grid(S.ctx, m->nslices), AT, 0, sx>>>(
        m->n, m->nslices, m->slice_w, m->cols, m->vals, m->dinv, b, x, S.omega, y, nullptr);
    KERNEL_CHECK();
    return NODAL_OK;
}

template <int MODE>
int cycle_sweep(Solver& S, const DLevel& L, const double* b, const double* xc, double* y, cudaStream_t sx) {
    const nodal_sell* m = L.sell;
    amg_cycle_sweep_kernel<MODE><<<amg_sell_grid(S.ctx, m->nslices), AT, 0, sx>>>(
        m->n, m->nslices, m->slice_w, m->cols, m->vals, m->dinv, b, S.omega, L.agg, xc, S.scale, y);
    KERNEL_CHECK();
    return NODAL_OK;
}

int cycle(Solver& S, const PcgDev* dev, const double* r0, double* u0, cudaStream_t sx) {
    nodal_ctx* ctx = S.ctx;
    const int ND = (int)S.lv.size() - 1;
    const bool fused = S.R == 1;
    for (int l = 0; l < ND; ++l) {
        DLevel& L = S.lv[l];
        const double* b = l == 0 ? r0 : L.b;
        if (fused) {
            NODAL_TRY(cycle_sweep<1>(S, L, b, nullptr, L.r, sx));
        } else {
            amg_jacobi0_kernel<<<amg_rows_grid(ctx, L.nloc), AT, 0, sx>>>(L.nloc, L.sell->dinv, b, S.omega, L.x);
            KERNEL_CHECK();
            NODAL_TRY(exchange(S, dev, 2 * l, L.halo, L.x_off, sx));
            NODAL_TRY(sweep<1>(S, L, b, L.x, L.r, sx));
        }
        amg_restrict_kernel<<<amg_rows_grid(ctx, L.nc), AT, 0, sx>>>(L.nc, L.pt_ptr, L.pt_idx, L.r, S.lv[l + 1].b);
        KERNEL_CHECK();
    }
    {
        DLevel& G = S.lv[ND];
        const double* b = ND == 0 ? r0 : G.b;
        if (S.R == 1) {
            NODAL_TRY(nodal_amg_apply(ctx, S.rep, b, S.xfull, sx));
        } else {
            if (S.p2p) {
                const int grid = (int)std::max<int64_t>(1, std::min<int64_t>(16, ((int64_t)G.nloc * S.R + 4095) / 4096));
                da_exchange_kernel<<<grid, 1024, 0, sx>>>(dev, AMG_SLOTS - 1, S.R, S.me, S.bfull_off, b, nullptr, nullptr,
                                                          S.gather_dest_dev, S.gather_need_dev, S.peer_dev, 1, G.nloc);
                KERNEL_CHECK();
            } else {
                CUDA_TRY(cudaMemcpyAsync(S.gather_stage + (size_t)S.R * S.gmax, b, sizeof(double) * (size_t)G.nloc,
                                         cudaMemcpyDeviceToDevice, sx));
                NCCL_TRY(g_nccl.AllGather(S.gather_stage + (size_t)S.R * S.gmax, S.gather_stage, S.gmax, ncclFloat64,
                                          S.d->comm, sx));
                for (int o = 0; o < S.R; ++o) {
                    const int32_t rows = S.rep_bounds[o + 1] - S.rep_bounds[o];
                    if (rows) CUDA_TRY(cudaMemcpyAsync(S.bfull + S.rep_bounds[o], S.gather_stage + (size_t)o * S.gmax,
                                                       sizeof(double) * (size_t)rows, cudaMemcpyDeviceToDevice, sx));
                }
            }
            NODAL_TRY(nodal_amg_apply(ctx, S.rep, S.bfull, S.xfull, sx));
        }
        if (ND == 0) {
            CUDA_TRY(cudaMemcpyAsync(u0, S.xfull + G.row0, sizeof(double) * (size_t)G.nloc, cudaMemcpyDeviceToDevice, sx));
            return NODAL_OK;
        }
    }
    for (int l = ND - 1; l >= 0; --l) {
        DLevel& L = S.lv[l];
        const double* b = l == 0 ? r0 : L.b;
        const double* xc = (l + 1 == ND) ? S.xfull + S.lv[ND].row0 : S.lv[l + 1].x;
        if (fused) {
            NODAL_TRY(cycle_sweep<2>(S, L, b, xc, l == 0 ? u0 : L.x, sx));
        } else {
            amg_prolong_kernel<<<amg_rows_grid(ctx, L.nloc), AT, 0, sx>>>(L.nloc, L.agg, xc, S.scale, L.x, L.r);
            KERNEL_CHECK();
            NODAL_TRY(exchange(S, dev, 2 * l + 1, L.halo, L.r_off, sx));
            NODAL_TRY(sweep<2>(S, L, b, L.r, l == 0 ? u0 : L.x, sx));
        }
    }
    return NODAL_OK;
}

}

extern "C" int nodal_dist_amg_pcg(nodal_ctx* ctx, nodal_dist* d, int32_t n_global, const int32_t* bounds_h,
                                  int64_t nnz, const int32_t* indptr, const int32_t* indices,
                                  const double* data, const double* rhs_local, double* x_local,
                                  const double* params, double rtol, int32_t maxit, int32_t* iters_h,
                                  double* relres_h, double* stats_h, void* stream) {
    NvtxRange nvtx_range("nodal_dist_amg_pcg");
    if (!ctx || !d || !bounds_h || !iters_h || !relres_h) return NODAL_BAD_ARG;
    *iters_h = 0;
    *relres_h = 0.0;
    if (stats_h) memset(stats_h, 0, 32 * sizeof(double));
    CUDA_TRY(cudaSetDevice(ctx->device));
    Solver S;
    S.ctx = ctx; S.d = d; S.R = d->nranks; S.me = d->rank; S.st = (cudaStream_t)stream;
    const int R = S.R, me = S.me;
// ... 82 lines not shown
            for (int o = 0; o < R; ++o) S.gmax = std::max(S.gmax, G.bounds[o + 1] - G.bounds[o]);
        }
        size_t bytes = AMG_HDR;
        auto place = [&](int64_t doubles) { const long long off = (long long)bytes; bytes += align_up((size_t)doubles * 8, 256); return off; };
        const long long u_off = place(S.lv[0].slot_len);
        const long long xs_off = place(S.lv[0].slot_len);
        for (int l = 0; l < ND; ++l) { S.lv[l].x_off = place(S.lv[l].slot_len); S.lv[l].r_off = place(S.lv[l].slot_len); }
        S.bfull_off = place((int64_t)S.rep_n + 2);
        bool usable = false;
        NODAL_TRY(peer_heap_ensure(ctx, d, &d->amg, bytes, AMG_HDR, st, &usable));
        S.p2p = usable;
        if (S.p2p) {
            S.base = d->amg.shm;
            S.peer_dev = d->amg.peer_dev;
        } else {
            local_buf = static_cast<char*>(ctx_pool_alloc(ctx, bytes));
            if (!local_buf) return NODAL_CUDA_ERROR;
            CUDA_TRY(cudaMemsetAsync(local_buf, 0, AMG_HDR, st));
            S.base = local_buf;
        }
        double* u = reinterpret_cast<double*>(S.base + u_off);
        for (int l = 0; l < ND; ++l) {
            DLevel& L = S.lv[l];
            L.x = reinterpret_cast<double*>(S.base + L.x_off);
            L.r = reinterpret_cast<double*>(S.base + L.r_off);
        }
        for (int l = 1; l <= ND; ++l) {
            S.lv[l].b = S.alloc<double>((size_t)S.lv[l].nloc + 2);
            if (!S.lv[l].b) return NODAL_CUDA_ERROR;
        }
        S.bfull = reinterpret_cast<double*>(S.base + S.bfull_off);
        S.xfull = S.alloc<double>((size_t)S.rep_n + 2);
        if (!S.xfull) return NODAL_CUDA_ERROR;
        if (R > 1) {
            std::vector<long long> gd(R, (long long)S.rep_bounds[me]);
            std::vector<int32_t> gn(R);
            for (int o = 0; o < R; ++o) gn[o] = S.rep_bounds[o + 1] - S.rep_bounds[o];
            S.gather_dest_dev = S.alloc<long long>((size_t)R);
            S.gather_need_dev = S.alloc<int32_t>((size_t)R);
            S.gather_stage = S.alloc<double>((size_t)(R + 1) * S.gmax + 2);
            if (!S.gather_dest_dev || !S.gather_need_dev || !S.gather_stage) return NODAL_CUDA_ERROR;
            CUDA_TRY(cudaMemcpyAsync(S.gather_dest_dev, gd.data(), sizeof(long long) * (size_t)R, cudaMemcpyHostToDevice, st));
            CUDA_TRY(cudaMemcpyAsync(S.gather_need_dev, gn.data(), sizeof(int32_t) * (size_t)R, cudaMemcpyHostToDevice, st));
            CUDA_TRY(cudaStreamSynchronize(st));
        }
        DLevel& F = S.lv[0];
        const int32_t n = F.nloc;
        const int gv = amg_rows_grid(ctx, n);
        const int gs = amg_sell_grid(ctx, F.sell->nslices);
        const int gmaxp = std::max(gv, gs) + 1;
        double* r = S.alloc<double>((size_t)n + 2);
        double* p = S.alloc<double>((size_t)n + 2);
        double* s = S.alloc<double>((size_t)n + 2);
        double* w = S.alloc<double>((size_t)n + 2);
        double* part = S.alloc<double>(4 * (size_t)gmaxp + 64);
        PcgDev* dev = S.alloc<PcgDev>(1);
        if (!r || !p || !s || !w || !part || !dev) return NODAL_CUDA_ERROR;
        double* part_g = part;
        double* part_d = part + gmaxp;
        double* part_rr = part + 2 * (size_t)gmaxp;
        double* part_bb = part + 3 * (size_t)gmaxp;
        double* SC = part + 4 * (size_t)gmaxp;
        CUDA_TRY(cudaMemsetAsync(dev, 0, sizeof(PcgDev), st));
        CUDA_TRY(cudaMemsetAsync(SC, 0, sizeof(double) * 32, st));
        const int use_mail = (S.p2p && R > 1) ? 1 : 0;

        auto allreduce = [&](int check_done, const double* a, int na, const double* b, int nb, const double* c, int nc,
                             const double* dd, int nd, double* out, int enforce, cudaStream_t sx) -> int {
            acg_allreduce_kernel<<<1, DA, 0, sx>>>(dev, check_done, a, na, b, nb, c, nc, dd, nd, R, me, S.peer_dev, use_mail,
                                                   out, enforce);
            KERNEL_CHECK();
            if (R > 1 && !use_mail) NCCL_TRY(g_nccl.AllReduce(out, out, 4, ncclFloat64, ncclSum, d->comm, sx));
            return NODAL_OK;
        };
        double* xstage = reinterpret_cast<double*>(S.base + xs_off);
        auto start = [&](int first) -> int {
            CUDA_TRY(cudaMemcpyAsync(xstage, x_local, sizeof(double) * (size_t)n, cudaMemcpyDeviceToDevice, st));
            NODAL_TRY(exchange(S, nullptr, AMG_SLOTS - 2, F.halo, xs_off, st));
            NODAL_TRY(sweep<1>(S, F, rhs_local, xstage, r, st));
            acg_start_kernel<<<gv, DA, 0, st>>>(n, rhs_local, r, p, s, part_rr, part_bb);
            KERNEL_CHECK();
            NODAL_TRY(cycle(S, nullptr, r, u, st));
            NODAL_TRY(exchange(S, nullptr, 2 * ND, F.halo, u_off, st));
            acg_spmv_dots_kernel<<<gs, DA, 0, st>>>(n, F.sell->nslices, F.sell->slice_w, F.sell->cols, F.sell->vals, u, r, w,
                                                    part_g, part_d);
            KERNEL_CHECK();
            NODAL_TRY(allreduce(0, part_g, gs, part_d, gs, part_rr, gv, part_bb, gv, SC, 0, st));
            acg_scalars_kernel<<<1, 32, 0, st>>>(dev, SC, rtol, maxit, first);
            KERNEL_CHECK();
            return NODAL_OK;
        };
        auto iteration = [&](int par, cudaStream_t sx) -> int {
            double* cur = SC + par * 4;
            double* nxt = SC + (par ^ 1) * 4;
            acg_vector_kernel<<<gv, DA, 0, sx>>>(dev, n, cur, nxt, x_local, r, p, s, u, w, part_rr);
            KERNEL_CHECK();
            NODAL_TRY(cycle(S, dev, r, u, sx));
            NODAL_TRY(exchange(S, dev, 2 * ND, F.halo, u_off, sx));
            acg_spmv_dots_kernel<<<gs, DA, 0, sx>>>(n, F.sell->nslices, F.sell->slice_w, F.sell->cols, F.sell->vals, u, r, w,
                                                    part_g, part_d);
            KERNEL_CHECK();
            NODAL_TRY(allreduce(1, part_g, gs, part_d, gs, part_rr, gv, nullptr, 0, nxt, 1, sx));
            return NODAL_OK;
        };
        nvtxRangePushA("amg first residual + cycle");
        const int start_rc = start(1);
        nvtxRangePop();
        NODAL_TRY(start_rc);
        const bool use_graph = getenv("NODAL_DIST_NO_GRAPH") == nullptr;
        if (use_graph) {
            const unsigned long long before = g_nodal_launches;
            CUDA_TRY(cudaStreamCreateWithFlags(&cap, cudaStreamNonBlocking));
            for (int par = 0; par < 2; ++par) {
                CUDA_TRY(cudaStreamBeginCapture(cap, cudaStreamCaptureModeThreadLocal));
                const int crc = iteration(par, cap);
                cudaError_t ce = cudaStreamEndCapture(cap, &graph[par]);
                if (crc != NODAL_OK) return crc;
                CUDA_TRY(ce);
                CUDA_TRY(cudaGraphInstantiate(&gexec[par], graph[par], 0));
            }
            launches_per_iter = (g_nodal_launches - before) / 2;
            g_nodal_launches = before;
        }
        CUDA_TRY(cudaEventRecord(ev1, st));
        phase.reset();
        phase.reset(new NvtxRange("amg-pcg iterations"));
        PcgDev* poll = reinterpret_cast<PcgDev*>(ctx->pinned);
        double last_true_rr = -1.0;
        int par = 0;
        for (;;) {
            int64_t k = 0;
            const int64_t max_iters = (int64_t)maxit + 4;
            for (;; ++k) {
                if (use_graph) {
                    CUDA_TRY(cudaGraphLaunch(gexec[par], st));
                    g_nodal_launches += launches_per_iter;
                } else {
                    NODAL_TRY(iteration(par, st));
                }
                par ^= 1;
                CUDA_TRY(cudaMemcpyAsync(&poll[k & 1], dev, sizeof(PcgDev), cudaMemcpyDeviceToHost, st));
                CUDA_TRY(cudaEventRecord(ev_poll[k & 1], st));
                if (R > 1 && !use_mail) {
                    CUDA_TRY(cudaEventSynchronize(ev_poll[k & 1]));
                    if (poll[k & 1].done) break;
                    if (k > max_iters) break;
                    continue;
                }
                if (k >= 1) {
                    CUDA_TRY(cudaEventSynchronize(ev_poll[(k - 1) & 1]));
                    if (poll[(k - 1) & 1].done) break;
                }
                if (k > max_iters) break;
            }
            CUDA_TRY(cudaStreamSynchronize(st));
            host = poll[k & 1];
            if (!host.done) host.status = NODAL_NOT_CONVERGED;
            if (host.status == NODAL_BREAKDOWN || host.status == NODAL_CUDA_ERROR) break;
            const int recurrence_status = host.status;
            const int iters_so_far = host.iters;
            NODAL_TRY(start(0));
            par = 0;
            CUDA_TRY(cudaMemcpyAsync(&poll[0], dev, sizeof(PcgDev), cudaMemcpyDeviceToHost, st));
            CUDA_TRY(cudaStreamSynchronize(st));
            host = poll[0];
            host.iters = iters_so_far;
            if (host.rr <= host.tol2) { host.status = NODAL_OK; break; }
            if (!(host.rr == host.rr)) { host.status = NODAL_BREAKDOWN; break; }
            if (recurrence_status == NODAL_NOT_CONVERGED || host.iters >= host.maxit) { host.status = NODAL_NOT_CONVERGED; break; }
            if (restarts >= 8 || (last_true_rr >= 0.0 && host.rr > 0.25 * last_true_rr)) { host.status = NODAL_NOT_CONVERGED; break; }
            last_true_rr = host.rr;
            ++restarts;
        }
        CUDA_TRY(cudaEventRecord(ev2, st));
        CUDA_TRY(cudaEventSynchronize(ev2));
        CUDA_TRY(cudaEventElapsedTime(&ms_setup, ev0, ev1));
        CUDA_TRY(cudaEventElapsedTime(&ms_solve, ev1, ev2));
        relres = host.bb > 0.0 ? sqrt(host.rr / host.bb) : 0.0;
        if (S.p2p) {
            unsigned long long err = 0;
            CUDA_TRY(cudaMemcpy(&err, &reinterpret_cast<AmgMail*>(S.base)->err, sizeof(err), cudaMemcpyDeviceToHost));
            if (err) {
// ... 48 lines not shown
```

nodal_b200/csrc/pcg_kernels.cuh:

```cuda
#pragma once
#include "sparse.cuh"

constexpr int PCG_THREADS = 256;
constexpr int PCG_CHUNK = 64;

struct PcgDev {
    double bb, tol2, rr;
    int iters, done, status, maxit;
};

__device__ __forceinline__ bool block_done(const int* done) {
    __shared__ int s_done;
    if (threadIdx.x == 0) s_done = *reinterpret_cast<const volatile int*>(done);
    __syncthreads();
    return s_done != 0;
}

template <int MINB>
static __global__ void __launch_bounds__(PCG_THREADS, MINB)
pcg_spmv_dot_sell_kernel(const PcgDev* __restrict__ dev, int32_t n, int32_t nslices,
                         const u32* __restrict__ slice_w, const int32_t* __restrict__ cols,
                         const double* __restrict__ vals, const double* __restrict__ p,
                         double* __restrict__ q, double* __restrict__ part_pq) {
    __shared__ double sm[40];
    if (block_done(&dev->done)) return;
    const int lane = threadIdx.x & 31;
    const int64_t warp = ((int64_t)blockIdx.x * blockDim.x + threadIdx.x) >> 5;
    const int64_t nwarps = ((int64_t)gridDim.x * blockDim.x) >> 5;
    double dot = 0.0;
    for (int64_t s = warp; s < nslices; s += nwarps) {
        const u32 w0 = slice_w[s];
        const int w = (int)(slice_w[s + 1] - w0);
        const int64_t base = (int64_t)w0 * 32 + lane;
        const double acc = sell_row_dot(cols, vals, base, w, p);
        const int64_t r = s * 32 + lane;
        if (r < n) {
            q[r] = acc;
            dot = fma(acc, __ldg(&p[r]), dot);
        }
    }
    dot = block_sum(dot, sm);
    if (threadIdx.x == 0) part_pq[blockIdx.x] = dot;
}

template <int TPR>
static __global__ void __launch_bounds__(PCG_THREADS)
pcg_spmv_dot_csr_kernel(const PcgDev* __restrict__ dev, int32_t n,
                        const int32_t* __restrict__ indptr, const int32_t* __restrict__ indices,
                        const double* __restrict__ data, const double* __restrict__ p,
                        double* __restrict__ q, double* __restrict__ part_pq) {
    __shared__ double sm[40];
    if (block_done(&dev->done)) return;
    constexpr int RPW = 32 / TPR;
    const int lane = threadIdx.x & 31, sub = lane & (TPR - 1);
    const int64_t warp = ((int64_t)blockIdx.x * blockDim.x + threadIdx.x) >> 5;
    const int64_t nwarps = ((int64_t)gridDim.x * blockDim.x) >> 5;
    double dot = 0.0;
    for (int64_t r0 = warp * RPW; r0 < n; r0 += nwarps * RPW) {
        const int64_t row = r0 + lane / TPR;
        double acc = 0.0;
        if (row < n) {
            const int32_t e = indptr[row + 1];
            for (int32_t j = indptr[row] + sub; j < e; j += TPR)
                acc = fma(data[j], __ldg(&p[indices[j]]), acc);
        }
#pragma unroll
        for (int o = TPR >> 1; o > 0; o >>= 1) acc += __shfl_xor_sync(0xffffffffu, acc, o);
        if (sub == 0 && row < n) {
            q[row] = acc;
            dot = fma(acc, __ldg(&p[row]), dot);
        }
    }
    dot = block_sum(dot, sm);
    if (threadIdx.x == 0) part_pq[blockIdx.x] = dot;
}

template <bool UNIT>
static __global__ void __launch_bounds__(PCG_THREADS)
pcg_update_kernel(PcgDev* __restrict__ dev, int32_t n, const double* __restrict__ part_pq, int g1,
                  const double* __restrict__ part_rz_prev, int g2, double* __restrict__ x,
                  const double* __restrict__ p, double* __restrict__ r,
                  const double* __restrict__ q, const double* __restrict__ dinv,
                  double* __restrict__ part_rz, double* __restrict__ part_rr) {
    __shared__ double sm[40];
    if (block_done(&dev->done)) return;
    double pq, rz, unused;
    if (g1 <= 8 * PCG_THREADS && g2 <= 8 * PCG_THREADS) {
        reduce_partials3(part_pq, g1, part_rz_prev, g2, nullptr, 0, sm, pq, rz, unused);
    } else {
        pq = reduce_partials(part_pq, g1, sm);
        rz = reduce_partials(part_rz_prev, g2, sm);
    }
    if (!(pq > 0.0)) {
        if (blockIdx.x == 0 && threadIdx.x == 0) { dev->done = 1; dev->status = NODAL_BREAKDOWN; }
        return;
    }
    const double alpha = rz / pq;
    double lrz = 0.0, lrr = 0.0;
    const int64_t n2 = n >> 1;
    const int64_t stride = (int64_t)gridDim.x * blockDim.x;
    double2* x2 = reinterpret_cast<double2*>(x);
    double2* r2 = reinterpret_cast<double2*>(r);
    const double2* p2 = reinterpret_cast<const double2*>(p);
    const double2* q2 = reinterpret_cast<const double2*>(q);
    const double2* d2 = reinterpret_cast<const double2*>(dinv);
    for (int64_t i = (int64_t)blockIdx.x * blockDim.x + threadIdx.x; i < n2; i += stride) {
        double2 xv = x2[i], rv = r2[i];
        const double2 pv = p2[i], qv = q2[i];
        xv.x = fma(alpha, pv.x, xv.x); xv.y = fma(alpha, pv.y, xv.y);
        rv.x = fma(-alpha, qv.x, rv.x); rv.y = fma(-alpha, qv.y, rv.y);
        x2[i] = xv; r2[i] = rv;
        if (!UNIT) {
            const double2 dv = d2[i];
            lrz = fma(rv.x * dv.x, rv.x, lrz); lrz = fma(rv.y * dv.y, rv.y, lrz);
        }
        lrr = fma(rv.x, rv.x, lrr); lrr = fma(rv.y, rv.y, lrr);
    }
// ... 94 lines not shown
    if (threadIdx.x == 0) {
        if (first) {
            dev->bb = bb;
            dev->tol2 = rtol * rtol * bb;
            dev->iters = 0;
            dev->maxit = maxit;
        }
        dev->rr = rr;
        dev->status = NODAL_OK;
        dev->done = 0;
        if (rr <= dev->tol2) dev->done = 1;
        else if (dev->iters >= dev->maxit) { dev->done = 1; dev->status = NODAL_NOT_CONVERGED; }
        else if (!(rr == rr)) { dev->done = 1; dev->status = NODAL_BREAKDOWN; }
    }
}

static __global__ void __launch_bounds__(PCG_THREADS)
csr_dinv_kernel(int32_t n, const int32_t* __restrict__ indptr, const int32_t* __restrict__ indices,
                const double* __restrict__ data, double* __restrict__ dinv) {
    for (int64_t r = (int64_t)blockIdx.x * blockDim.x + threadIdx.x; r < n;
         r += (int64_t)gridDim.x * blockDim.x) {
        double dg = 0.0;
        for (int32_t j = indptr[r]; j < indptr[r + 1]; ++j)
            if (indices[j] == r) dg += data[j];
        dinv[r] = dg != 0.0 ? 1.0 / dg : 1.0;
    }
}


static __global__ void __launch_bounds__(PCG_THREADS)
pcg_scale_factors_kernel(int32_t n, const int32_t* __restrict__ indptr, const int32_t* __restrict__ indices,
                         const double* __restrict__ data, double* __restrict__ sc, int* __restrict__ flag) {
    for (int64_t r = (int64_t)blockIdx.x * blockDim.x + threadIdx.x; r < n;
         r += (int64_t)gridDim.x * blockDim.x) {
        double dg = 0.0;
        for (int32_t j = indptr[r]; j < indptr[r + 1]; ++j)
            if (indices[j] == r) dg += data[j];
        if (dg > 0.0) sc[r] = 1.0 / sqrt(dg);
        else { sc[r] = 1.0; *flag = 1; }
    }
}

static __global__ void __launch_bounds__(PCG_THREADS)
pcg_scale_vec_kernel(int32_t n, const double* in, const double* __restrict__ sc, double* out, int mode) {
    for (int64_t i = (int64_t)blockIdx.x * blockDim.x + threadIdx.x; i < n;
         i += (int64_t)gridDim.x * blockDim.x)
        out[i] = mode ? in[i] / sc[i] : in[i] * sc[i];
}

static __global__ void __launch_bounds__(PCG_THREADS)
pcg_unscaled_norm_kernel(int32_t n, const double* __restrict__ rhat, const double* __restrict__ sc,
                         const double* __restrict__ b, double* __restrict__ part_rr,
                         double* __restrict__ part_bb) {
    __shared__ double sm[40];
    double lrr = 0.0, lbb = 0.0;
    for (int64_t i = (int64_t)blockIdx.x * blockDim.x + threadIdx.x; i < n;
         i += (int64_t)gridDim.x * blockDim.x) {
        const double rv = rhat[i] / sc[i];
        lrr = fma(rv, rv, lrr);
        lbb = fma(b[i], b[i], lbb);
    }
    lrr = block_sum(lrr, sm);
    lbb = block_sum(lbb, sm);
    if (threadIdx.x == 0) { part_rr[blockIdx.x] = lrr; part_bb[blockIdx.x] = lbb; }
}

struct Mat {
    const nodal_sell* sell = nullptr;
    int32_t n = 0;
    int64_t nnz = 0;
    const int32_t* indptr = nullptr;
    const int32_t* indices = nullptr;
    const double* data = nullptr;
    int tpr = 4;
    int g1 = 1;
    int minb = 5;
};

static inline int launch_k1(const Mat& A, const PcgDev* dev, const double* p, double* q, double* part_pq,
              cudaStream_t st) {
    if (A.sell) {
#define GOS(M)                                                                                 \
    pcg_spmv_dot_sell_kernel<M><<<A.g1, PCG_THREADS, 0, st>>>(dev, A.n, A.sell->nslices,       \
                                                              A.sell->slice_w, A.sell->cols,   \
                                                              A.sell->vals, p, q, part_pq)
        switch (A.minb) {
            case 5: GOS(5); break;
            case 6: GOS(6); break;
            default: GOS(4); break;
        }
#undef GOS
    } else {
#define GO(T)                                                                                  \
    pcg_spmv_dot_csr_kernel<T><<<A.g1, PCG_THREADS, 0, st>>>(dev, A.n, A.indptr, A.indices,    \
                                                             A.data, p, q, part_pq)
        switch (A.tpr) {
            case 2: GO(2); break;
            case 4: GO(4); break;
            case 8: GO(8); break;
            case 16: GO(16); break;
            default: GO(32); break;
        }
#undef GO
    }
    KERNEL_CHECK();
    return NODAL_OK;
}
```

nodal_b200/csrc/sparse.cuh:

```cuda
#pragma once
#include "common.cuh"

struct nodal_sell {
    nodal_ctx* ctx = nullptr;
    int device = 0;
    int32_t n = 0;
    int32_t nslices = 0;
    int64_t padded = 0;
    int64_t nnz = 0;
    u32* slice_w = nullptr;
    int32_t* cols = nullptr;
    double* vals = nullptr;
    size_t store_bytes = 0;
    double* dinv = nullptr;
};

int sell_from_csr(nodal_ctx* ctx, int32_t n, int64_t nnz, const int32_t* indptr,
                  const int32_t* indices, const double* data, nodal_sell** out, cudaStream_t st,
                  const double* sc = nullptr);
void sell_free(nodal_sell* m);
int sell_set_l2_window(nodal_ctx* ctx, const nodal_sell* m, cudaStream_t st);
void sell_clear_l2_window(cudaStream_t st);

int csr_spmv_launch(nodal_ctx* ctx, int32_t n, int64_t nnz, const int32_t* indptr,
                    const int32_t* indices, const double* data, const double* x, double* y,
                    cudaStream_t st);
int csr_spmv_rows_launch(nodal_ctx* ctx, int32_t rows, const int32_t* indptr, const int32_t* indices,
                         const double* data, const double* x, double* y, int32_t shape_n, int64_t shape_nnz,
                         cudaStream_t st);

#ifdef __CUDACC__
#include "amg_cycle_core.cuh"

struct SellLoad {
    const double* __restrict__ x;
    __device__ __forceinline__ double operator()(int32_t c) const { return __ldg(&x[c]); }
};

template <int W, class G>
__device__ __forceinline__ double sell_dot_fixed(const int32_t* __restrict__ cols,
                                                 const double* __restrict__ vals, int64_t base,
                                                 const G& gather, double acc) {
    int32_t c[W];
    double v[W], xv[W];
#pragma unroll
    for (int i = 0; i < W; ++i) {
        c[i] = cols[base + (int64_t)i * 32];
        v[i] = vals[base + (int64_t)i * 32];
    }
#pragma unroll
    for (int i = 0; i < W; ++i) xv[i] = gather(c[i]);
#pragma unroll
    for (int i = 0; i < W; ++i) acc = amg_dot_step(v[i], xv[i], acc);
    return acc;
}

template <class G>
__device__ __forceinline__ double sell_row_gather(const int32_t* __restrict__ cols,
                                                  const double* __restrict__ vals, int64_t base, int w,
                                                  const G& x) {
    double acc = 0.0;
    int k = 0;
    for (; k + 8 <= w; k += 8) acc = sell_dot_fixed<8>(cols, vals, base + (int64_t)k * 32, x, acc);
    const int64_t b = base + (int64_t)k * 32;
    switch (w - k) {
        case 7: acc = sell_dot_fixed<7>(cols, vals, b, x, acc); break;
        case 6: acc = sell_dot_fixed<6>(cols, vals, b, x, acc); break;
        case 5: acc = sell_dot_fixed<5>(cols, vals, b, x, acc); break;
        case 4: acc = sell_dot_fixed<4>(cols, vals, b, x, acc); break;
        case 3: acc = sell_dot_fixed<3>(cols, vals, b, x, acc); break;
        case 2: acc = sell_dot_fixed<2>(cols, vals, b, x, acc); break;
        case 1: acc = sell_dot_fixed<1>(cols, vals, b, x, acc); break;
        default: break;
    }
    return acc;
}

__device__ __forceinline__ double sell_row_dot(const int32_t* __restrict__ cols,
                                               const double* __restrict__ vals, int64_t base, int w,
                                               const double* __restrict__ x) {
    return sell_row_gather(cols, vals, base, w, SellLoad{x});
}
#endif
```

nodal_b200/csrc/spmv.cu:

```cuda
#include <algorithm>

#include "sparse.cuh"

constexpr int SPMV_THREADS = 256;

template <int TPR>
__global__ void __launch_bounds__(SPMV_THREADS)
csr_spmv_kernel(int32_t n, const int32_t* __restrict__ indptr, const int32_t* __restrict__ indices,
                const double* __restrict__ data, const double* __restrict__ x,
                double* __restrict__ y) {
    constexpr int RPW = 32 / TPR;
    const int lane = threadIdx.x & 31, sub = lane & (TPR - 1);
    const int64_t warp = ((int64_t)blockIdx.x * blockDim.x + threadIdx.x) >> 5;
    const int64_t nwarps = ((int64_t)gridDim.x * blockDim.x) >> 5;
    for (int64_t r0 = warp * RPW; r0 < n; r0 += nwarps * RPW) {
        const int64_t row = r0 + lane / TPR;
        double acc = 0.0;
        if (row < n) {
            const int32_t e = indptr[row + 1];
            for (int32_t j = indptr[row] + sub; j < e; j += TPR)
                acc = fma(data[j], __ldg(&x[indices[j]]), acc);
        }
#pragma unroll
        for (int o = TPR >> 1; o > 0; o >>= 1) acc += __shfl_xor_sync(0xffffffffu, acc, o);
        if (sub == 0 && row < n) y[row] = acc;
    }
}

static int pick_tpr(int32_t n, int64_t nnz) {
    const double mean = n > 0 ? (double)nnz / n : 1.0;
    if (mean <= 2.5) return 2;
    if (mean <= 6.0) return 4;
    if (mean <= 12.0) return 8;
    if (mean <= 24.0) return 16;
    return 32;
}

int csr_spmv_launch(nodal_ctx* ctx, int32_t n, int64_t nnz, const int32_t* indptr,
                    const int32_t* indices, const double* data, const double* x, double* y,
                    cudaStream_t st) {
    return csr_spmv_rows_launch(ctx, n, indptr, indices, data, x, y, n, nnz, st);
}

int csr_spmv_rows_launch(nodal_ctx* ctx, int32_t n, const int32_t* indptr, const int32_t* indices,
                         const double* data, const double* x, double* y, int32_t shape_n, int64_t shape_nnz,
                         cudaStream_t st) {
    if (n == 0) return NODAL_OK;
    const int tpr = pick_tpr(shape_n, shape_nnz);
    int64_t blocks = ((int64_t)n * tpr + SPMV_THREADS - 1) / SPMV_THREADS;
    const int64_t cap = (int64_t)ctx->num_sms * 8;
    const int grid = (int)(blocks < cap ? blocks : cap);
#define GO(T) csr_spmv_kernel<T><<<grid, SPMV_THREADS, 0, st>>>(n, indptr, indices, data, x, y)
    switch (tpr) {
        case 2: GO(2); break;
        case 4: GO(4); break;
        case 8: GO(8); break;
        case 16: GO(16); break;
        default: GO(32); break;
    }
#undef GO
    KERNEL_CHECK();
    return NODAL_OK;
}

extern "C" int nodal_spmv(nodal_ctx* ctx, int32_t n, int64_t nnz, const int32_t* indptr,
                          const int32_t* indices, const double* data, const double* x, double* y,
                          void* stream) {
    if (!ctx || n < 0) return NODAL_BAD_ARG;
    CUDA_TRY(cudaSetDevice(ctx->device));
    return csr_spmv_launch(ctx, n, nnz, indptr, indices, data, x, y, (cudaStream_t)stream);
}

__global__ void __launch_bounds__(SPMV_THREADS)
sell_widths_kernel(int32_t n, int32_t nslices, const int32_t* __restrict__ indptr,
                   u32* __restrict__ slice_w) {
    const int lane = threadIdx.x & 31;
    const int64_t warp = ((int64_t)blockIdx.x * blockDim.x + threadIdx.x) >> 5;
    const int64_t nwarps = ((int64_t)gridDim.x * blockDim.x) >> 5;
    for (int64_t s = warp; s < nslices; s += nwarps) {
        const int64_t r = s * 32 + lane;
        u32 len = 0;
        if (r < n) len = (u32)(indptr[r + 1] - indptr[r]);
#pragma unroll
        for (int o = 16; o > 0; o >>= 1) len = max(len, __shfl_xor_sync(0xffffffffu, len, o));
        if (lane == 0) slice_w[s] = len;
    }
}

__global__ void __launch_bounds__(SPMV_THREADS)
sell_fill_kernel(int32_t n, int32_t nslices, const int32_t* __restrict__ indptr,
                 const int32_t* __restrict__ indices, const double* __restrict__ data,
                 const u32* __restrict__ slice_w, const double* __restrict__ sc,
                 int32_t* __restrict__ cols, double* __restrict__ vals, double* __restrict__ dinv) {
    const int lane = threadIdx.x & 31;
    const int64_t warp = ((int64_t)blockIdx.x * blockDim.x + threadIdx.x) >> 5;
    const int64_t nwarps = ((int64_t)gridDim.x * blockDim.x) >> 5;
    for (int64_t s = warp; s < nslices; s += nwarps) {
        const int64_t r = s * 32 + lane;
        const u32 w0 = slice_w[s], w = slice_w[s + 1] - w0;
        int32_t b = 0, e = 0;
        if (r < n) { b = indptr[r]; e = indptr[r + 1]; }
        double diag = 0.0;
        const int64_t base = (int64_t)w0 * 32 + lane;
        for (u32 k = 0; k < w; ++k) {
            int32_t c = r < n ? (int32_t)r : 0;
            double v = 0.0;
            if (b + (int32_t)k < e) {
                c = indices[b + k];
                v = data[b + k];
                if (sc) v = (v * sc[r]) * sc[c];
                if (c == r) diag += v;
            }
            cols[base + (int64_t)k * 32] = c;
            vals[base + (int64_t)k * 32] = v;
        }
        if (r < n) dinv[r] = diag != 0.0 ? 1.0 / diag : 1.0;
    }
}

void sell_free(nodal_sell* m) {
    if (!m) return;
    cudaSetDevice(m->device);
    ctx_pool_free(m->ctx, m->slice_w);
    ctx_pool_free(m->ctx, m->vals);
    ctx_pool_free(m->ctx, m->dinv);
    delete m;
}

int sell_from_csr(nodal_ctx* ctx, int32_t n, int64_t nnz, const int32_t* indptr,
                  const int32_t* indices, const double* data, nodal_sell** out, cudaStream_t st,
                  const double* sc) {
    *out = nullptr;
    nodal_sell* m = new nodal_sell();
    m->ctx = ctx;
    m->device = ctx->device;
    m->n = n;
    m->nnz = nnz;
    m->nslices = (n + 31) / 32;
    const int64_t ns = m->nslices;
    int rc = NODAL_OK;
    auto fail = [&](int code) { sell_free(m); return code; };
#define CT(expr)                                                                             \
    do {                                                                                     \
        cudaError_t _e = (expr);                                                             \
        if (_e != cudaSuccess) {                                                             \
            nodal_set_error("%s:%d: %s -> %s", __FILE__, __LINE__, #expr,                    \
                            cudaGetErrorString(_e));                                         \
            return fail(NODAL_CUDA_ERROR);                                                   \
        }                                                                                    \
    } while (0)
#define PA(field, type, bytes)                                                               \
    do {                                                                                     \
        m->field = static_cast<type*>(ctx_pool_alloc(ctx, (bytes)));                         \
        if (!m->field) {                                                                     \
            nodal_set_error("%s:%d: out of device memory (%zu bytes)", __FILE__, __LINE__,   \
                            (size_t)(bytes));                                                \
            return fail(NODAL_CUDA_ERROR);                                                   \
        }                                                                                    \
    } while (0)
    PA(slice_w, u32, sizeof(u32) * (size_t)(ns + 1));
    PA(dinv, double, sizeof(double) * (size_t)(n > 0 ? n : 1));
    CT(cudaMemsetAsync(m->slice_w, 0, sizeof(u32) * (size_t)(ns + 1), st));
    if (n == 0) { *out = m; return NODAL_OK; }
    const int64_t cap = (int64_t)ctx->num_sms * 8;
    const int64_t want = (ns * 32 + SPMV_THREADS - 1) / SPMV_THREADS;
    const int grid = (int)(want < cap ? want : cap);
    sell_widths_kernel<<<grid, SPMV_THREADS, 0, st>>>(n, m->nslices, indptr, m->slice_w);
    CT(cudaGetLastError());
    rc = ctx_reserve(ctx, scan_scratch_bytes(ns + 1) + 4096);
    if (rc != NODAL_OK) return fail(rc);
    u32* tot = carve<u32>(ctx, 16);
    rc = scan_exclusive_u32(ctx, m->slice_w, m->slice_w, ns + 1, tot, st);
    if (rc != NODAL_OK) return fail(rc);
    u32* host_tot = reinterpret_cast<u32*>(ctx->pinned);
    CT(cudaMemcpyAsync(host_tot, tot, sizeof(u32), cudaMemcpyDeviceToHost, st));
    CT(cudaStreamSynchronize(st));
    m->padded = (int64_t)host_tot[0] * 32;
    const size_t alloc = (size_t)(m->padded > 0 ? m->padded : 32);
    PA(vals, double, sizeof(double) * alloc + sizeof(int32_t) * alloc);
    m->cols = reinterpret_cast<int32_t*>(m->vals + alloc);
    m->store_bytes = (sizeof(double) + sizeof(int32_t)) * alloc;
#undef PA
    sell_fill_kernel<<<grid, SPMV_THREADS, 0, st>>>(n, m->nslices, indptr, indices, data,
                                                    m->slice_w, sc, m->cols, m->vals, m->dinv);
    CT(cudaGetLastError());
#undef CT
    *out = m;
    return NODAL_OK;
}

__global__ void __launch_bounds__(SPMV_THREADS, 5)
sell_spmv_kernel(int32_t n, int32_t nslices, const u32* __restrict__ slice_w,
                 const int32_t* __restrict__ cols, const double* __restrict__ vals,
                 const double* __restrict__ x, double* __restrict__ y) {
    const int lane = threadIdx.x & 31;
    const int64_t warp = ((int64_t)blockIdx.x * blockDim.x + threadIdx.x) >> 5;
    const int64_t nwarps = ((int64_t)gridDim.x * blockDim.x) >> 5;
    for (int64_t s = warp; s < nslices; s += nwarps) {
        const u32 w0 = slice_w[s];
        const int w = (int)(slice_w[s + 1] - w0);
        const int64_t base = (int64_t)w0 * 32 + lane;
        const double acc = sell_row_dot(cols, vals, base, w, x);
        const int64_t r = s * 32 + lane;
        if (r < n) y[r] = acc;
    }
}

extern "C" int nodal_sell_create(nodal_ctx* ctx, int32_t n, int64_t nnz, const int32_t* indptr,
                                 const int32_t* indices, const double* data, nodal_sell** out,
                                 void* stream) {
    if (!ctx || n < 0 || !out) return NODAL_BAD_ARG;
    CUDA_TRY(cudaSetDevice(ctx->device));
    return sell_from_csr(ctx, n, nnz, indptr, indices, data, out, (cudaStream_t)stream, nullptr);
}

extern "C" int nodal_sell_destroy(nodal_sell* m) {
    sell_free(m);
    return NODAL_OK;
}

extern "C" int64_t nodal_sell_padded_nnz(const nodal_sell* m) { return m ? m->padded : 0; }

extern "C" int nodal_sell_spmv(nodal_ctx* ctx, const nodal_sell* m, const double* x, double* y,
                               void* stream) {
    if (!ctx || !m) return NODAL_BAD_ARG;
    if (m->n == 0) return NODAL_OK;
    CUDA_TRY(cudaSetDevice(ctx->device));
    const int64_t want = ((int64_t)m->nslices * 32 + SPMV_THREADS - 1) / SPMV_THREADS;
    const int64_t cap = (int64_t)ctx->num_sms * 5;
    sell_spmv_kernel<<<(int)(want < cap ? want : cap), SPMV_THREADS, 0, (cudaStream_t)stream>>>(
        m->n, m->nslices, m->slice_w, m->cols, m->vals, x, y);
    KERNEL_CHECK();
    return NODAL_OK;
}

int sell_set_l2_window(nodal_ctx* ctx, const nodal_sell* m, cudaStream_t st) {
    if (!m || !m->vals || !getenv("NODAL_L2_WINDOW")) return NODAL_OK;
    cudaDeviceProp prop;
    CUDA_TRY(cudaGetDeviceProperties(&prop, ctx->device));
    if (prop.persistingL2CacheMaxSize <= 0 || prop.accessPolicyMaxWindowSize <= 0) return NODAL_OK;
    const size_t persist = (size_t)prop.persistingL2CacheMaxSize;
    CUDA_TRY(cudaDeviceSetLimit(cudaLimitPersistingL2CacheSize, persist));
    cudaStreamAttrValue attr;
    memset(&attr, 0, sizeof(attr));
    const size_t window = std::min<size_t>(m->store_bytes, (size_t)prop.accessPolicyMaxWindowSize);
    attr.accessPolicyWindow.base_ptr = m->vals;
    attr.accessPolicyWindow.num_bytes = window;
    attr.accessPolicyWindow.hitRatio = (float)std::min(1.0, 0.85 * (double)persist / (double)window);
    attr.accessPolicyWindow.hitProp = cudaAccessPropertyPersisting;
    attr.accessPolicyWindow.missProp = cudaAccessPropertyStreaming;
    CUDA_TRY(cudaStreamSetAttribute(st, cudaStreamAttributeAccessPolicyWindow, &attr));
    return NODAL_OK;
}

void sell_clear_l2_window(cudaStream_t st) {
    if (!getenv("NODAL_L2_WINDOW")) return;
    cudaStreamAttrValue attr;
    memset(&attr, 0, sizeof(attr));
    attr.accessPolicyWindow.num_bytes = 0;
    cudaStreamSetAttribute(st, cudaStreamAttributeAccessPolicyWindow, &attr);
    cudaCtxResetPersistingL2Cache();
}
```

Before: 145.2 million.

## Compress stencil SELL slices by storing shared column offsets instead of per-row indices

```diff
diff --git a/__graft_entry__.py b/__graft_entry__.py
--- a/__graft_entry__.py
+++ b/__graft_entry__.py
@@ -17,6 +17,8 @@
     sources_host.sources_host_lib()
     import amg_cycle_host
     amg_cycle_host.amg_cycle_host_lib()
+    import sell_host
+    sell_host.sell_host_lib()
     ref_nodal = os.path.join(os.environ.get("NODAL_REFERENCE", "/root/reference"), "nodal")
     if os.path.isdir(ref_nodal) and not os.path.isfile(os.path.join(ROOT, "baseline", "_ref", "nodal", "nodal.py")):
         subprocess.call([sys.executable, os.path.join(ROOT, "baseline", "install_ref.py")])
diff --git a/include/nodal_b200.h b/include/nodal_b200.h
--- a/include/nodal_b200.h
+++ b/include/nodal_b200.h
@@ -63,7 +63,9 @@
                       const int32_t* indices, const double* data, nodal_sell** out, void* stream);
 int nodal_sell_destroy(nodal_sell* m);
 int64_t nodal_sell_padded_nnz(const nodal_sell* m);
+int64_t nodal_sell_stencil_nnz(const nodal_sell* m);
 int nodal_sell_spmv(nodal_ctx* ctx, const nodal_sell* m, const double* x, double* y, void* stream);
+int nodal_sell_spmm(nodal_ctx* ctx, const nodal_sell* m, int32_t K, const double* x, double* y, void* stream);
 
 int nodal_pcg(nodal_ctx* ctx, int32_t n, int64_t nnz, const int32_t* indptr,
               const int32_t* indices, const double* data, const double* rhs, double* x,
diff --git a/nodal_b200/_lib.py b/nodal_b200/_lib.py
--- a/nodal_b200/_lib.py
+++ b/nodal_b200/_lib.py
@@ -29,7 +29,9 @@
     "nodal_sell_create": (C.c_int, [_vp, _i32, _i64, _vp, _vp, _vp, C.POINTER(_vp), _vp]),
     "nodal_sell_destroy": (C.c_int, [_vp]),
     "nodal_sell_padded_nnz": (_i64, [_vp]),
+    "nodal_sell_stencil_nnz": (_i64, [_vp]),
     "nodal_sell_spmv": (C.c_int, [_vp, _vp, _vp, _vp, _vp]),
+    "nodal_sell_spmm": (C.c_int, [_vp, _vp, _i32, _vp, _vp, _vp]),
     "nodal_pcg": (C.c_int, [_vp, _i32, _i64, _vp, _vp, _vp, _vp, _vp, _f64, _i32, _i32,
                             C.POINTER(_i32), C.POINTER(_f64), C.POINTER(_f64), _vp]),
     "nodal_gmres": (C.c_int, [_vp, _i32, _i64, _vp, _vp, _vp, _vp, _vp, _f64, _i32, _i32,
diff --git a/nodal_b200/csrc/amg.cu b/nodal_b200/csrc/amg.cu
--- a/nodal_b200/csrc/amg.cu
+++ b/nodal_b200/csrc/amg.cu
@@ -293,7 +293,7 @@
                double* part, cudaStream_t st) {
     const nodal_sell* m = V.sell;
     amg_sell_kernel<MODE><<<sell_grid(h->ctx, m->nslices), AT, 0, st>>>(
-        m->n, m->nslices, m->slice_w, m->cols, m->vals, m->dinv, b, x, h->omega, y, part);
+        m->n, m->nslices, sell_view(m), m->dinv, b, x, h->omega, y, part);
     KERNEL_CHECK();
     return NODAL_OK;
 }
@@ -303,7 +303,7 @@
                 cudaStream_t st) {
     const nodal_sell* m = V.sell;
     amg_cycle_sweep_kernel<MODE><<<sell_grid(h->ctx, m->nslices), AT, 0, st>>>(
-        m->n, m->nslices, m->slice_w, m->cols, m->vals, m->dinv, b, h->omega, V.agg, xc, h->scale, y);
+        m->n, m->nslices, sell_view(m), m->dinv, b, h->omega, V.agg, xc, h->scale, y);
     KERNEL_CHECK();
     return NODAL_OK;
 }
diff --git a/nodal_b200/csrc/amg_kernels.cuh b/nodal_b200/csrc/amg_kernels.cuh
--- a/nodal_b200/csrc/amg_kernels.cuh
+++ b/nodal_b200/csrc/amg_kernels.cuh
@@ -125,9 +125,7 @@
 
 template <int MODE>
 static __global__ void __launch_bounds__(AT, 5)
-amg_sell_kernel(int32_t n, int32_t nslices, const u32* __restrict__ slice_w,
-                const int32_t* __restrict__ cols, const double* __restrict__ vals,
-                const double* __restrict__ dinv, const double* __restrict__ b,
+amg_sell_kernel(int32_t n, int32_t nslices, const SellView A, const double* __restrict__ dinv, const double* __restrict__ b,
                 const double* __restrict__ x, double omega, double* __restrict__ y,
                 double* __restrict__ part) {
     __shared__ double red[33];
@@ -136,9 +134,7 @@
     const int64_t nwarps = ((int64_t)gridDim.x * blockDim.x) >> 5;
     double dot = 0.0;
     for (int64_t s = warp; s < nslices; s += nwarps) {
-        const u32 w0 = slice_w[s];
-        const int w = (int)(slice_w[s + 1] - w0);
-        const double acc = sell_row_dot(cols, vals, (int64_t)w0 * 32 + lane, w, x);
+        const double acc = sell_slice_dot(A, s, lane, x);
         const int64_t r = s * 32 + lane;
         if (r < n) {
             if (MODE == 0) { y[r] = acc; dot = fma(x[r], acc, dot); }
@@ -190,9 +186,7 @@
 
 template <int MODE>
 static __global__ void __launch_bounds__(AT, 5)
-amg_cycle_sweep_kernel(int32_t n, int32_t nslices, const u32* __restrict__ slice_w,
-                       const int32_t* __restrict__ cols, const double* __restrict__ vals,
-                       const double* __restrict__ dinv, const double* __restrict__ b, double omega,
+amg_cycle_sweep_kernel(int32_t n, int32_t nslices, const SellView A, const double* __restrict__ dinv, const double* __restrict__ b, double omega,
                        const int32_t* __restrict__ agg, const double* __restrict__ xc, double scale,
                        double* __restrict__ y) {
     const int lane = threadIdx.x & 31;
@@ -201,16 +195,13 @@
     const JacobiStartAt x0{dinv, b, omega};
     const ProlongatedAt xa{x0, agg, xc, scale};
     for (int64_t s = warp; s < nslices; s += nwarps) {
-        const u32 w0 = slice_w[s];
-        const int w = (int)(slice_w[s + 1] - w0);
-        const int64_t base = (int64_t)w0 * 32 + lane;
         const int64_t r = s * 32 + lane;
         if (MODE == 1) {
-            const double acc = sell_row_gather(cols, vals, base, w, x0);
+            const double acc = sell_slice_gather(A, s, lane, x0);
             if (r < n) y[r] = amg_residual(b[r], acc);
         }
         if (MODE == 2) {
-            const double acc = sell_row_gather(cols, vals, base, w, xa);
+            const double acc = sell_slice_gather(A, s, lane, xa);
             if (r < n) y[r] = amg_jacobi_update(omega, dinv[r], b[r], acc, xa((int32_t)r));
         }
     }
diff --git a/nodal_b200/csrc/amg_multi.cu b/nodal_b200/csrc/amg_multi.cu
--- a/nodal_b200/csrc/amg_multi.cu
+++ b/nodal_b200/csrc/amg_multi.cu
@@ -7,15 +7,15 @@
 
 constexpr int MK = 8;
 
-template <int W>
-__device__ __forceinline__ void sell_dot_fixed_multi(const int32_t* __restrict__ cols, const double* __restrict__ vals,
-                                                     int64_t base, const double* __restrict__ x, int64_t stride, int K,
+template <int W, class C>
+__device__ __forceinline__ void sell_dot_fixed_multi(const C& col, const double* __restrict__ vals, int64_t base,
+                                                     const double* __restrict__ x, int64_t stride, int K,
                                                      double* acc) {
     int32_t c[W];
     double v[W];
 #pragma unroll
     for (int i = 0; i < W; ++i) {
-        c[i] = cols[base + (int64_t)i * 32];
+        c[i] = col[i];
         v[i] = vals[base + (int64_t)i * 32];
     }
 #pragma unroll
@@ -30,24 +30,44 @@
     }
 }
 
-__device__ __forceinline__ void sell_row_dot_multi(const int32_t* __restrict__ cols, const double* __restrict__ vals,
-                                                   int64_t base, int w, const double* __restrict__ x, int64_t stride,
-                                                   int K, double* acc) {
+template <class C>
+__device__ __forceinline__ void sell_row_dot_multi(const C& col, const double* __restrict__ vals, int64_t base,
+                                                   int w, const double* __restrict__ x, int64_t stride, int K,
+                                                   double* acc) {
     int k = 0;
-    for (; k + 4 <= w; k += 4) sell_dot_fixed_multi<4>(cols, vals, base + (int64_t)k * 32, x, stride, K, acc);
+    for (; k + 4 <= w; k += 4) sell_dot_fixed_multi<4>(col + k, vals, base + (int64_t)k * 32, x, stride, K, acc);
+    const C ck = col + k;
     const int64_t b = base + (int64_t)k * 32;
     switch (w - k) {
-        case 3: sell_dot_fixed_multi<3>(cols, vals, b, x, stride, K, acc); break;
-        case 2: sell_dot_fixed_multi<2>(cols, vals, b, x, stride, K, acc); break;
-        case 1: sell_dot_fixed_multi<1>(cols, vals, b, x, stride, K, acc); break;
+        case 3: sell_dot_fixed_multi<3>(ck, vals, b, x, stride, K, acc); break;
+        case 2: sell_dot_fixed_multi<2>(ck, vals, b, x, stride, K, acc); break;
+        case 1: sell_dot_fixed_multi<1>(ck, vals, b, x, stride, K, acc); break;
         default: break;
     }
+}
+
+struct SellColsAny {
+    const int32_t* __restrict__ p;
+    int32_t step, add;
+    __device__ __forceinline__ int32_t operator[](int i) const { return p[(int64_t)i * step] + add; }
+    __device__ __forceinline__ SellColsAny operator+(int k) const { return {p + (int64_t)k * step, step, add}; }
+};
+
+__device__ __forceinline__ void sell_slice_dot_multi(const SellView& A, int64_t s, int lane,
+                                                     const double* __restrict__ x, int64_t stride, int K,
+                                                     double* acc) {
+    const u32 w0 = A.slice_w[s];
+    const int w = (int)(A.slice_w[s + 1] - w0);
+    const u32 d = A.slice_c[s];
+    const bool st = d & SELL_STENCIL;
+    const SellColsAny col = st ? SellColsAny{A.offs + (d & ~SELL_STENCIL), 1, (int32_t)(s * 32 + lane)}
+                               : SellColsAny{A.cols + (int64_t)d * 32 + lane, 32, 0};
+    sell_row_dot_multi(col, A.vals, (int64_t)w0 * 32 + lane, w, x, stride, K, acc);
 }
 
 template <int MODE>
 __global__ void __launch_bounds__(AT, 3)
-amgm_sell_kernel(int32_t n, int32_t nslices, const u32* __restrict__ slice_w, const int32_t* __restrict__ cols,
-                 const double* __restrict__ vals, const double* __restrict__ dinv, const double* __restrict__ b,
+amgm_sell_kernel(int32_t n, int32_t nslices, const SellView A, const double* __restrict__ dinv, const double* __restrict__ b,
                  const double* __restrict__ x, double omega, double* __restrict__ y, double* __restrict__ part, int K,
                  int nparts) {
     __shared__ double red[33];
@@ -58,12 +78,10 @@
 #pragma unroll
     for (int k = 0; k < MK; ++k) dot[k] = 0.0;
     for (int64_t s = warp; s < nslices; s += nwarps) {
-        const u32 w0 = slice_w[s];
-        const int w = (int)(slice_w[s + 1] - w0);
         double acc[MK];
 #pragma unroll
         for (int k = 0; k < MK; ++k) acc[k] = 0.0;
-        sell_row_dot_multi(cols, vals, (int64_t)w0 * 32 + lane, w, x, n, K, acc);
+        sell_slice_dot_multi(A, s, lane, x, n, K, acc);
         const int64_t r = s * 32 + lane;
         if (r < n) {
             const double di = MODE == 2 ? dinv[r] : 0.0;
@@ -210,7 +228,7 @@
           int nparts, cudaStream_t st) {
     const nodal_sell* m = V.sell;
     amgm_sell_kernel<MODE><<<amg_sell_grid(h->ctx, m->nslices), AT, 0, st>>>(
-        m->n, m->nslices, m->slice_w, m->cols, m->vals, m->dinv, b, x, h->omega, y, part, K, nparts);
+        m->n, m->nslices, sell_view(m), m->dinv, b, x, h->omega, y, part, K, nparts);
     KERNEL_CHECK();
     return NODAL_OK;
 }
@@ -246,6 +264,20 @@
     return NODAL_OK;
 }
 
+}
+
+extern "C" int nodal_sell_spmm(nodal_ctx* ctx, const nodal_sell* m, int32_t K, const double* x, double* y,
+                               void* stream) {
+    if (!ctx || !m || K < 1 || K > MK) return NODAL_BAD_ARG;
+    if (m->n == 0) return NODAL_OK;
+    CUDA_TRY(cudaSetDevice(ctx->device));
+    const int grid = amg_sell_grid(ctx, m->nslices);
+    NODAL_TRY(ctx_reserve(ctx, sizeof(double) * (size_t)K * grid + 4096));
+    double* part = carve<double>(ctx, (size_t)K * grid);
+    amgm_sell_kernel<0><<<grid, AT, 0, (cudaStream_t)stream>>>(m->n, m->nslices, sell_view(m), m->dinv, nullptr, x,
+                                                              0.0, y, part, K, grid);
+    KERNEL_CHECK();
+    return NODAL_OK;
 }
 
 extern "C" int nodal_amg_pcg_multi(nodal_ctx* ctx, nodal_amg* h, int32_t K, const double* rhs, double* x, double rtol,
diff --git a/nodal_b200/csrc/dist.cu b/nodal_b200/csrc/dist.cu
--- a/nodal_b200/csrc/dist.cu
+++ b/nodal_b200/csrc/dist.cu
@@ -607,8 +607,7 @@
 
 __global__ void __launch_bounds__(PCG_THREADS, 5)
 dist_spmv_allreduce_sell_kernel(PcgDev* __restrict__ dev, int32_t n, int32_t nslices,
-                                const u32* __restrict__ slice_w, const int32_t* __restrict__ cols,
-                                const double* __restrict__ vals, const double* __restrict__ u,
+                                const SellView A, const double* __restrict__ u,
                                 double* __restrict__ w, double* part_d, const double* __restrict__ part_g,
                                 const double* __restrict__ part_rr, int cnt_v, DistSync* sy,
                                 unsigned long long* seq, int R, int me,
@@ -630,10 +629,7 @@
     const int64_t nwarps = ((int64_t)gridDim.x * blockDim.x) >> 5;
     double dot = 0.0;
     for (int64_t s = warp; s < nslices; s += nwarps) {
-        const u32 w0 = slice_w[s];
-        const int wd = (int)(slice_w[s + 1] - w0);
-        const int64_t base = (int64_t)w0 * 32 + lane;
-        const double acc = sell_row_dot(cols, vals, base, wd, u);
+        const double acc = sell_slice_dot(A, s, lane, u);
         const int64_t row = s * 32 + lane;
         if (row < n) {
             w[row] = acc;
@@ -1118,7 +1114,7 @@
                         bmask_dev, d->pcg.peer_dev);
                 KERNEL_CHECK();
                 dist_spmv_allreduce_sell_kernel<<<A.g1, PCG_THREADS, 0, sx>>>(
-                    dev, nloc, sell->nslices, sell->slice_w, sell->cols, sell->vals, ext, w, part_d, part_g,
+                    dev, nloc, sell->nslices, sell_view(sell), ext, w, part_d, part_g,
                     part_rr, g2, sy, d->pcg.seq, R, me, d->pcg.peer_dev, nxt);
                 KERNEL_CHECK();
                 return NODAL_OK;
diff --git a/nodal_b200/csrc/dist_amg.cu b/nodal_b200/csrc/dist_amg.cu
--- a/nodal_b200/csrc/dist_amg.cu
+++ b/nodal_b200/csrc/dist_amg.cu
@@ -217,8 +217,7 @@
 }
 
 __global__ void __launch_bounds__(DA, 5)
-acg_spmv_dots_kernel(int32_t n, int32_t nslices, const u32* __restrict__ slice_w, const int32_t* __restrict__ cols,
-                     const double* __restrict__ vals, const double* __restrict__ u, const double* __restrict__ r,
+acg_spmv_dots_kernel(int32_t n, int32_t nslices, const SellView A, const double* __restrict__ u, const double* __restrict__ r,
                      double* __restrict__ w, double* __restrict__ part_g, double* __restrict__ part_d) {
     __shared__ double sm[40];
     const int lane = threadIdx.x & 31;
@@ -226,9 +225,7 @@
     const int64_t nwarps = ((int64_t)gridDim.x * blockDim.x) >> 5;
     double lg = 0.0, ld = 0.0;
     for (int64_t s = warp; s < nslices; s += nwarps) {
-        const u32 w0 = slice_w[s];
-        const int wd = (int)(slice_w[s + 1] - w0);
-        const double acc = sell_row_dot(cols, vals, (int64_t)w0 * 32 + lane, wd, u);
+        const double acc = sell_slice_dot(A, s, lane, u);
         const int64_t row = s * 32 + lane;
         if (row < n) {
             const double uv = __ldg(&u[row]);
@@ -763,7 +760,7 @@
 int sweep(Solver& S, const DLevel& L, const double* b, const double* x, double* y, cudaStream_t sx) {
     const nodal_sell* m = L.sell;
     amg_sell_kernel<MODE><<<amg_sell_grid(S.ctx, m->nslices), AT, 0, sx>>>(
-        m->n, m->nslices, m->slice_w, m->cols, m->vals, m->dinv, b, x, S.omega, y, nullptr);
+        m->n, m->nslices, sell_view(m), m->dinv, b, x, S.omega, y, nullptr);
     KERNEL_CHECK();
     return NODAL_OK;
 }
@@ -772,7 +769,7 @@
 int cycle_sweep(Solver& S, const DLevel& L, const double* b, const double* xc, double* y, cudaStream_t sx) {
     const nodal_sell* m = L.sell;
     amg_cycle_sweep_kernel<MODE><<<amg_sell_grid(S.ctx, m->nslices), AT, 0, sx>>>(
-        m->n, m->nslices, m->slice_w, m->cols, m->vals, m->dinv, b, S.omega, L.agg, xc, S.scale, y);
+        m->n, m->nslices, sell_view(m), m->dinv, b, S.omega, L.agg, xc, S.scale, y);
     KERNEL_CHECK();
     return NODAL_OK;
 }
@@ -1021,7 +1018,7 @@
             KERNEL_CHECK();
             NODAL_TRY(cycle(S, nullptr, r, u, st));
             NODAL_TRY(exchange(S, nullptr, 2 * ND, F.halo, u_off, st));
-            acg_spmv_dots_kernel<<<gs, DA, 0, st>>>(n, F.sell->nslices, F.sell->slice_w, F.sell->cols, F.sell->vals, u, r, w,
+            acg_spmv_dots_kernel<<<gs, DA, 0, st>>>(n, F.sell->nslices, sell_view(F.sell), u, r, w,
                                                     part_g, part_d);
             KERNEL_CHECK();
             NODAL_TRY(allreduce(0, part_g, gs, part_d, gs, part_rr, gv, part_bb, gv, SC, 0, st));
@@ -1036,7 +1033,7 @@
             KERNEL_CHECK();
             NODAL_TRY(cycle(S, dev, r, u, sx));
             NODAL_TRY(exchange(S, dev, 2 * ND, F.halo, u_off, sx));
-            acg_spmv_dots_kernel<<<gs, DA, 0, sx>>>(n, F.sell->nslices, F.sell->slice_w, F.sell->cols, F.sell->vals, u, r, w,
+            acg_spmv_dots_kernel<<<gs, DA, 0, sx>>>(n, F.sell->nslices, sell_view(F.sell), u, r, w,
                                                     part_g, part_d);
             KERNEL_CHECK();
             NODAL_TRY(allreduce(1, part_g, gs, part_d, gs, part_rr, gv, nullptr, 0, nxt, 1, sx));
diff --git a/nodal_b200/csrc/pcg_kernels.cuh b/nodal_b200/csrc/pcg_kernels.cuh
--- a/nodal_b200/csrc/pcg_kernels.cuh
+++ b/nodal_b200/csrc/pcg_kernels.cuh
@@ -19,8 +19,7 @@
 template <int MINB>
 static __global__ void __launch_bounds__(PCG_THREADS, MINB)
 pcg_spmv_dot_sell_kernel(const PcgDev* __restrict__ dev, int32_t n, int32_t nslices,
-                         const u32* __restrict__ slice_w, const int32_t* __restrict__ cols,
-                         const double* __restrict__ vals, const double* __restrict__ p,
+                         const SellView A, const double* __restrict__ p,
                          double* __restrict__ q, double* __restrict__ part_pq) {
     __shared__ double sm[40];
     if (block_done(&dev->done)) return;
@@ -29,10 +28,7 @@
     const int64_t nwarps = ((int64_t)gridDim.x * blockDim.x) >> 5;
     double dot = 0.0;
     for (int64_t s = warp; s < nslices; s += nwarps) {
-        const u32 w0 = slice_w[s];
-        const int w = (int)(slice_w[s + 1] - w0);
-        const int64_t base = (int64_t)w0 * 32 + lane;
-        const double acc = sell_row_dot(cols, vals, base, w, p);
+        const double acc = sell_slice_dot(A, s, lane, p);
         const int64_t r = s * 32 + lane;
         if (r < n) {
             q[r] = acc;
@@ -293,8 +289,7 @@
     if (A.sell) {
 #define GOS(M)                                                                                 \
     pcg_spmv_dot_sell_kernel<M><<<A.g1, PCG_THREADS, 0, st>>>(dev, A.n, A.sell->nslices,       \
-                                                              A.sell->slice_w, A.sell->cols,   \
-                                                              A.sell->vals, p, q, part_pq)
+                                                              sell_view(A.sell), p, q, part_pq)
         switch (A.minb) {
             case 5: GOS(5); break;
             case 6: GOS(6); break;
diff --git a/nodal_b200/csrc/sell_core.cuh b/nodal_b200/csrc/sell_core.cuh
--- /dev/null
+++ b/nodal_b200/csrc/sell_core.cuh
@@ -0,0 +1,33 @@
+#pragma once
+#include <stdint.h>
+
+#if defined(__CUDACC__)
+#define SELLC_HD __host__ __device__ __forceinline__
+#define SELLC_MEMBER __host__ __device__ __forceinline__
+#else
+#define SELLC_HD static inline
+#define SELLC_MEMBER inline
+#endif
+
+constexpr uint32_t SELL_STENCIL = 0x80000000u;
+
+SELLC_HD bool sell_slice_full(int64_t s, int64_t n) { return s * 32 + 32 <= n; }
+
+struct SellColsExplicit {
+    const int32_t* __restrict__ p;
+    SELLC_MEMBER int32_t operator[](int i) const { return p[(int64_t)i * 32]; }
+    SELLC_MEMBER SellColsExplicit operator+(int k) const { return {p + (int64_t)k * 32}; }
+};
+
+struct SellColsStencil {
+    const int32_t* __restrict__ off;
+    int32_t row;
+    SELLC_MEMBER int32_t operator[](int i) const { return row + off[i]; }
+    SELLC_MEMBER SellColsStencil operator+(int k) const { return {off + k, row}; }
+};
+
+SELLC_HD int32_t sell_entry_col(uint32_t desc, const int32_t* cols, const int32_t* offs, int64_t s, int l,
+                                int k) {
+    if (desc & SELL_STENCIL) return SellColsStencil{offs + (desc & ~SELL_STENCIL), (int32_t)(s * 32 + l)}[k];
+    return SellColsExplicit{cols + (int64_t)desc * 32 + l}[k];
+}
diff --git a/nodal_b200/csrc/sparse.cuh b/nodal_b200/csrc/sparse.cuh
--- a/nodal_b200/csrc/sparse.cuh
+++ b/nodal_b200/csrc/sparse.cuh
@@ -1,5 +1,6 @@
 #pragma once
 #include "common.cuh"
+#include "sell_core.cuh"
 
 struct nodal_sell {
     nodal_ctx* ctx = nullptr;
@@ -8,12 +9,24 @@
     int32_t nslices = 0;
     int64_t padded = 0;
     int64_t nnz = 0;
+    int64_t stencil_nnz = 0;
     u32* slice_w = nullptr;
+    u32* slice_c = nullptr;
+    double* vals = nullptr;
     int32_t* cols = nullptr;
-    double* vals = nullptr;
+    int32_t* offs = nullptr;
     size_t store_bytes = 0;
     double* dinv = nullptr;
 };
+
+struct SellView {
+    const u32* __restrict__ slice_w;
+    const u32* __restrict__ slice_c;
+    const int32_t* __restrict__ cols;
+    const int32_t* __restrict__ offs;
+    const double* __restrict__ vals;
+};
+static inline SellView sell_view(const nodal_sell* m) { return {m->slice_w, m->slice_c, m->cols, m->offs, m->vals}; }
 
 int sell_from_csr(nodal_ctx* ctx, int32_t n, int64_t nnz, const int32_t* indptr,
                   const int32_t* indices, const double* data, nodal_sell** out, cudaStream_t st,
@@ -37,15 +50,14 @@
     __device__ __forceinline__ double operator()(int32_t c) const { return __ldg(&x[c]); }
 };
 
-template <int W, class G>
-__device__ __forceinline__ double sell_dot_fixed(const int32_t* __restrict__ cols,
-                                                 const double* __restrict__ vals, int64_t base,
+template <int W, class C, class G>
+__device__ __forceinline__ double sell_dot_fixed(const C& col, const double* __restrict__ vals, int64_t base,
                                                  const G& gather, double acc) {
     int32_t c[W];
     double v[W], xv[W];
 #pragma unroll
     for (int i = 0; i < W; ++i) {
-        c[i] = cols[base + (int64_t)i * 32];
+        c[i] = col[i];
         v[i] = vals[base + (int64_t)i * 32];
     }
 #pragma unroll
@@ -55,30 +67,41 @@
     return acc;
 }
 
-template <class G>
-__device__ __forceinline__ double sell_row_gather(const int32_t* __restrict__ cols,
-                                                  const double* __restrict__ vals, int64_t base, int w,
-                                                  const G& x) {
+template <class C, class G>
+__device__ __forceinline__ double sell_row_gather(const C& col, const double* __restrict__ vals, int64_t base,
+                                                  int w, const G& x) {
     double acc = 0.0;
     int k = 0;
-    for (; k + 8 <= w; k += 8) acc = sell_dot_fixed<8>(cols, vals, base + (int64_t)k * 32, x, acc);
+    for (; k + 8 <= w; k += 8) acc = sell_dot_fixed<8>(col + k, vals, base + (int64_t)k * 32, x, acc);
+    const C ck = col + k;
     const int64_t b = base + (int64_t)k * 32;
     switch (w - k) {
-        case 7: acc = sell_dot_fixed<7>(cols, vals, b, x, acc); break;
-        case 6: acc = sell_dot_fixed<6>(cols, vals, b, x, acc); break;
-        case 5: acc = sell_dot_fixed<5>(cols, vals, b, x, acc); break;
-        case 4: acc = sell_dot_fixed<4>(cols, vals, b, x, acc); break;
-        case 3: acc = sell_dot_fixed<3>(cols, vals, b, x, acc); break;
-        case 2: acc = sell_dot_fixed<2>(cols, vals, b, x, acc); break;
-        case 1: acc = sell_dot_fixed<1>(cols, vals, b, x, acc); break;
+        case 7: acc = sell_dot_fixed<7>(ck, vals, b, x, acc); break;
+        case 6: acc = sell_dot_fixed<6>(ck, vals, b, x, acc); break;
+        case 5: acc = sell_dot_fixed<5>(ck, vals, b, x, acc); break;
+        case 4: acc = sell_dot_fixed<4>(ck, vals, b, x, acc); break;
+        case 3: acc = sell_dot_fixed<3>(ck, vals, b, x, acc); break;
+        case 2: acc = sell_dot_fixed<2>(ck, vals, b, x, acc); break;
+        case 1: acc = sell_dot_fixed<1>(ck, vals, b, x, acc); break;
         default: break;
     }
     return acc;
 }
 
-__device__ __forceinline__ double sell_row_dot(const int32_t* __restrict__ cols,
-                                               const double* __restrict__ vals, int64_t base, int w,
-                                               const double* __restrict__ x) {
-    return sell_row_gather(cols, vals, base, w, SellLoad{x});
+template <class G>
+__device__ __forceinline__ double sell_slice_gather(const SellView& A, int64_t s, int lane, const G& x) {
+    const u32 w0 = A.slice_w[s];
+    const int w = (int)(A.slice_w[s + 1] - w0);
+    const u32 d = A.slice_c[s];
+    const int64_t base = (int64_t)w0 * 32 + lane;
+    if (d & SELL_STENCIL)
+        return sell_row_gather(SellColsStencil{A.offs + (d & ~SELL_STENCIL), (int32_t)(s * 32 + lane)}, A.vals, base,
+                               w, x);
+    return sell_row_gather(SellColsExplicit{A.cols + (int64_t)d * 32 + lane}, A.vals, base, w, x);
+}
+
+__device__ __forceinline__ double sell_slice_dot(const SellView& A, int64_t s, int lane,
+                                                 const double* __restrict__ x) {
+    return sell_slice_gather(A, s, lane, SellLoad{x});
 }
 #endif
diff --git a/nodal_b200/csrc/spmv.cu b/nodal_b200/csrc/spmv.cu
--- a/nodal_b200/csrc/spmv.cu
+++ b/nodal_b200/csrc/spmv.cu
@@ -73,35 +73,48 @@
 
 __global__ void __launch_bounds__(SPMV_THREADS)
 sell_widths_kernel(int32_t n, int32_t nslices, const int32_t* __restrict__ indptr,
-                   u32* __restrict__ slice_w) {
+                   const int32_t* __restrict__ indices, u32* __restrict__ slice_w, u32* __restrict__ ew) {
     const int lane = threadIdx.x & 31;
     const int64_t warp = ((int64_t)blockIdx.x * blockDim.x + threadIdx.x) >> 5;
     const int64_t nwarps = ((int64_t)gridDim.x * blockDim.x) >> 5;
     for (int64_t s = warp; s < nslices; s += nwarps) {
         const int64_t r = s * 32 + lane;
         u32 len = 0;
-        if (r < n) len = (u32)(indptr[r + 1] - indptr[r]);
+        int32_t b = 0;
+        if (r < n) { b = indptr[r]; len = (u32)(indptr[r + 1] - b); }
+        u32 w = len;
 #pragma unroll
-        for (int o = 16; o > 0; o >>= 1) len = max(len, __shfl_xor_sync(0xffffffffu, len, o));
-        if (lane == 0) slice_w[s] = len;
+        for (int o = 16; o > 0; o >>= 1) w = max(w, __shfl_xor_sync(0xffffffffu, w, o));
+        bool st = sell_slice_full(s, n) && w > 0 && __all_sync(0xffffffffu, len == w);
+        for (u32 k = 0; st && k < w; ++k) {
+            const int32_t d = indices[b + k] - (int32_t)r;
+            st = __all_sync(0xffffffffu, d == __shfl_sync(0xffffffffu, d, 0));
+        }
+        if (lane == 0) { slice_w[s] = w; ew[s] = st ? 0u : w; }
     }
 }
 
 __global__ void __launch_bounds__(SPMV_THREADS)
 sell_fill_kernel(int32_t n, int32_t nslices, const int32_t* __restrict__ indptr,
                  const int32_t* __restrict__ indices, const double* __restrict__ data,
-                 const u32* __restrict__ slice_w, const double* __restrict__ sc,
-                 int32_t* __restrict__ cols, double* __restrict__ vals, double* __restrict__ dinv) {
+                 const u32* __restrict__ slice_w, const u32* __restrict__ ew, u32* __restrict__ slice_c,
+                 const double* __restrict__ sc, int32_t* __restrict__ cols, int32_t* __restrict__ offs,
+                 double* __restrict__ vals, double* __restrict__ dinv) {
     const int lane = threadIdx.x & 31;
     const int64_t warp = ((int64_t)blockIdx.x * blockDim.x + threadIdx.x) >> 5;
     const int64_t nwarps = ((int64_t)gridDim.x * blockDim.x) >> 5;
     for (int64_t s = warp; s < nslices; s += nwarps) {
         const int64_t r = s * 32 + lane;
         const u32 w0 = slice_w[s], w = slice_w[s + 1] - w0;
+        const u32 e0 = slice_c[s];
+        const bool stencil = w > 0 && ew[s] == 0;
+        const u32 o0 = w0 - e0;
+        __syncwarp();
         int32_t b = 0, e = 0;
         if (r < n) { b = indptr[r]; e = indptr[r + 1]; }
         double diag = 0.0;
         const int64_t base = (int64_t)w0 * 32 + lane;
+        const int64_t cbase = (int64_t)e0 * 32 + lane;
         for (u32 k = 0; k < w; ++k) {
             int32_t c = r < n ? (int32_t)r : 0;
             double v = 0.0;
@@ -111,10 +124,12 @@
                 if (sc) v = (v * sc[r]) * sc[c];
                 if (c == r) diag += v;
             }
-            cols[base + (int64_t)k * 32] = c;
+            if (!stencil) cols[cbase + (int64_t)k * 32] = c;
+            else if (lane == 0) offs[o0 + k] = c - (int32_t)r;
             vals[base + (int64_t)k * 32] = v;
         }
         if (r < n) dinv[r] = diag != 0.0 ? 1.0 / diag : 1.0;
+        if (lane == 0) slice_c[s] = stencil ? (SELL_STENCIL | o0) : e0;
     }
 }
 
@@ -122,6 +137,7 @@
     if (!m) return;
     cudaSetDevice(m->device);
     ctx_pool_free(m->ctx, m->slice_w);
+    ctx_pool_free(m->ctx, m->slice_c);
     ctx_pool_free(m->ctx, m->vals);
     ctx_pool_free(m->ctx, m->dinv);
     delete m;
@@ -159,30 +175,44 @@
         }                                                                                    \
     } while (0)
     PA(slice_w, u32, sizeof(u32) * (size_t)(ns + 1));
+    PA(slice_c, u32, sizeof(u32) * (size_t)(ns + 1));
     PA(dinv, double, sizeof(double) * (size_t)(n > 0 ? n : 1));
     CT(cudaMemsetAsync(m->slice_w, 0, sizeof(u32) * (size_t)(ns + 1), st));
+    CT(cudaMemsetAsync(m->slice_c, 0, sizeof(u32) * (size_t)(ns + 1), st));
     if (n == 0) { *out = m; return NODAL_OK; }
+    rc = ctx_reserve(ctx, 2 * scan_scratch_bytes(ns + 1) + align_up(sizeof(u32) * (size_t)(ns + 1), 256) + 4096);
+    if (rc != NODAL_OK) return fail(rc);
+    u32* tot = carve<u32>(ctx, 16);
+    u32* ew = carve<u32>(ctx, (size_t)(ns + 1));
+    CT(cudaMemsetAsync(ew + ns, 0, sizeof(u32), st));
     const int64_t cap = (int64_t)ctx->num_sms * 8;
     const int64_t want = (ns * 32 + SPMV_THREADS - 1) / SPMV_THREADS;
     const int grid = (int)(want < cap ? want : cap);
-    sell_widths_kernel<<<grid, SPMV_THREADS, 0, st>>>(n, m->nslices, indptr, m->slice_w);
+    sell_widths_kernel<<<grid, SPMV_THREADS, 0, st>>>(n, m->nslices, indptr, indices, m->slice_w, ew);
     CT(cudaGetLastError());
-    rc = ctx_reserve(ctx, scan_scratch_bytes(ns + 1) + 4096);
-    if (rc != NODAL_OK) return fail(rc);
-    u32* tot = carve<u32>(ctx, 16);
     rc = scan_exclusive_u32(ctx, m->slice_w, m->slice_w, ns + 1, tot, st);
     if (rc != NODAL_OK) return fail(rc);
+    rc = scan_exclusive_u32(ctx, ew, m->slice_c, ns + 1, tot + 1, st);
+    if (rc != NODAL_OK) return fail(rc);
     u32* host_tot = reinterpret_cast<u32*>(ctx->pinned);
-    CT(cudaMemcpyAsync(host_tot, tot, sizeof(u32), cudaMemcpyDeviceToHost, st));
+    CT(cudaMemcpyAsync(host_tot, tot, 2 * sizeof(u32), cudaMemcpyDeviceToHost, st));
     CT(cudaStreamSynchronize(st));
-    m->padded = (int64_t)host_tot[0] * 32;
+    if (host_tot[0] >= SELL_STENCIL) {
+        nodal_set_error("sell_from_csr: %u k-steps exceed the SELL-32 descriptor range", host_tot[0]);
+        return fail(NODAL_BAD_ARG);
+    }
+    const int64_t ksteps = host_tot[0], explicit_ksteps = host_tot[1];
+    m->padded = ksteps * 32;
+    m->stencil_nnz = (ksteps - explicit_ksteps) * 32;
     const size_t alloc = (size_t)(m->padded > 0 ? m->padded : 32);
-    PA(vals, double, sizeof(double) * alloc + sizeof(int32_t) * alloc);
+    const size_t ncols = (size_t)explicit_ksteps * 32, noffs = (size_t)(ksteps - explicit_ksteps);
+    m->store_bytes = sizeof(double) * alloc + sizeof(int32_t) * (ncols + noffs);
+    PA(vals, double, m->store_bytes);
     m->cols = reinterpret_cast<int32_t*>(m->vals + alloc);
-    m->store_bytes = (sizeof(double) + sizeof(int32_t)) * alloc;
+    m->offs = m->cols + ncols;
 #undef PA
-    sell_fill_kernel<<<grid, SPMV_THREADS, 0, st>>>(n, m->nslices, indptr, indices, data,
-                                                    m->slice_w, sc, m->cols, m->vals, m->dinv);
+    sell_fill_kernel<<<grid, SPMV_THREADS, 0, st>>>(n, m->nslices, indptr, indices, data, m->slice_w, ew,
+                                                    m->slice_c, sc, m->cols, m->offs, m->vals, m->dinv);
     CT(cudaGetLastError());
 #undef CT
     *out = m;
@@ -190,17 +220,13 @@
 }
 
 __global__ void __launch_bounds__(SPMV_THREADS, 5)
-sell_spmv_kernel(int32_t n, int32_t nslices, const u32* __restrict__ slice_w,
-                 const int32_t* __restrict__ cols, const double* __restrict__ vals,
-                 const double* __restrict__ x, double* __restrict__ y) {
+sell_spmv_kernel(int32_t n, int32_t nslices, const SellView A, const double* __restrict__ x,
+                 double* __restrict__ y) {
     const int lane = threadIdx.x & 31;
     const int64_t warp = ((int64_t)blockIdx.x * blockDim.x + threadIdx.x) >> 5;
     const int64_t nwarps = ((int64_t)gridDim.x * blockDim.x) >> 5;
     for (int64_t s = warp; s < nslices; s += nwarps) {
-        const u32 w0 = slice_w[s];
-        const int w = (int)(slice_w[s + 1] - w0);
-        const int64_t base = (int64_t)w0 * 32 + lane;
-        const double acc = sell_row_dot(cols, vals, base, w, x);
+        const double acc = sell_slice_dot(A, s, lane, x);
         const int64_t r = s * 32 + lane;
         if (r < n) y[r] = acc;
     }
@@ -220,6 +246,8 @@
 }
 
 extern "C" int64_t nodal_sell_padded_nnz(const nodal_sell* m) { return m ? m->padded : 0; }
+
+extern "C" int64_t nodal_sell_stencil_nnz(const nodal_sell* m) { return m ? m->stencil_nnz : 0; }
 
 extern "C" int nodal_sell_spmv(nodal_ctx* ctx, const nodal_sell* m, const double* x, double* y,
                                void* stream) {
@@ -229,7 +257,7 @@
     const int64_t want = ((int64_t)m->nslices * 32 + SPMV_THREADS - 1) / SPMV_THREADS;
     const int64_t cap = (int64_t)ctx->num_sms * 5;
     sell_spmv_kernel<<<(int)(want < cap ? want : cap), SPMV_THREADS, 0, (cudaStream_t)stream>>>(
-        m->n, m->nslices, m->slice_w, m->cols, m->vals, x, y);
+        m->n, m->nslices, sell_view(m), x, y);
     KERNEL_CHECK();
     return NODAL_OK;
 }
```

Result: faster. 147.9 million (median of 6 runs) (+1.9%).
